# AbrahamSanders/realtime-codec-agent

Measured on NVIDIA B200. Metric: encode audio-sec/sec, higher is better.
Workload: dtype bf16

## Files before the change

### include/magicodec_b200.h

```cpp
#ifndef MAGICODEC_B200_H_
#define MAGICODEC_B200_H_

#include <stdint.h>

#ifdef __cplusplus
extern "C" {
#endif

#define MC_VERSION 100

enum {
  MC_OK = 0,
  MC_ERR_ARG = -1,
  MC_ERR_ARCH = -2,
  MC_ERR_CUDA = -3,
  MC_ERR_STATE = -4,
  MC_ERR_NOMEM = -5
};

typedef struct mc_handle mc_handle;
typedef void* mc_stream_t;

#define MC_MAX_CONVS 8

typedef struct mc_spec {
  int32_t sample_rate;
  int32_t n_convs;
  int32_t conv_channels[MC_MAX_CONVS];
  int32_t conv_strides[MC_MAX_CONVS];
  int32_t d_model, n_heads, ffn_dim;
  int32_t enc_layers, dec_layers;
  int32_t window_left, window_right;
  float norm_eps;
  int32_t codebook_size, codebook_dim;
  int32_t max_positions;
} mc_spec;

int mc_version(void);
const char* mc_last_error(const mc_handle* h);

int mc_create(const mc_spec* spec, int device, mc_handle** out);
int mc_destroy(mc_handle* h);

int mc_set_tensor(mc_handle* h, const char* name, const void* dev_ptr, int64_t numel);
int mc_finalize(mc_handle* h);

int mc_encode(mc_handle* h, const float* wav, int64_t ld, int32_t B, int32_t T, int32_t keep_last_frames,
              int64_t* codes, float* margin, float* z_e, mc_stream_t stream);

int mc_decode(mc_handle* h, const int64_t* codes, int32_t B, int32_t F, int32_t keep_last_samples, float* wav,
              mc_stream_t stream);
int mc_decode_latents(mc_handle* h, const float* z_q, int32_t B, int32_t F, int32_t keep_last_samples,
                      float* wav, mc_stream_t stream);

int mc_vq_search(mc_handle* h, const float* z, int32_t M, int64_t* codes, float* margin, mc_stream_t stream);

int mc_codebook(mc_handle* h, float* out, mc_stream_t stream);

int mc_op_gemm_fused(mc_handle* h, const void* A, const void* W, const float* bias, int32_t M, int32_t N, int32_t K, int32_t act,
                     int32_t out_mode, void* out, const float* row_stats, int32_t row_stats_n, void* xb_out, const float* xb_gamma,
                     float* stat_out, int32_t rope_cols, int32_t rope_period, int32_t block_n, mc_stream_t stream);
int mc_op_rowstats(mc_handle* h, const float* x, const float* gamma, void* xb_out, float* stat_out, int32_t M, int32_t d,
                   mc_stream_t stream);

int64_t mc_debug_trace(mc_handle* h, void* dev_buf, int64_t capacity_records);

enum { MC_PCM_U8 = 0, MC_PCM_S16 = 1, MC_PCM_S24 = 2, MC_PCM_S32 = 3, MC_PCM_F32 = 4, MC_PCM_F64 = 5, MC_PCM_ULAW = 6, MC_PCM_ALAW = 7 };
int mc_op_pcm_to_f32(mc_handle* h, const void* pcm, int32_t format, int32_t big_endian, int32_t channels, int64_t frames,
                     int32_t mix_mono, float* out, int64_t out_ld, mc_stream_t stream);
int mc_op_resample(mc_handle* h, const float* in, int64_t in_ld, int32_t channels, int64_t n_in, int32_t up, int32_t down,
                   const float* taps, int32_t n_taps, int64_t pre_remove, float* out, int64_t out_ld, int64_t n_out,
                   mc_stream_t stream);

int mc_flac_info(const uint8_t* data, int64_t n, int32_t* sample_rate, int32_t* channels, int32_t* bits, int64_t* total_samples);
int mc_flac_decode(const uint8_t* data, int64_t n, void* out, int64_t capacity_frames, int64_t* decoded);

typedef struct mc_stream mc_stream;
int mc_stream_create(mc_handle* h, int32_t channels, int32_t context_samples, int32_t max_chunk_samples, mc_stream** out);
int mc_stream_destroy(mc_stream* s);
int mc_stream_reset(mc_stream* s);
int mc_stream_reset_part(mc_stream* s, int32_t audio, int32_t codes);
int mc_stream_load_audio(mc_stream* s, const float* audio, int32_t n);
int mc_stream_load_codes(mc_stream* s, const int64_t* codes, int32_t n);
int mc_stream_push_audio(mc_stream* s, const float* chunk, int32_t n, int32_t keep_frames, int64_t* codes_out,
                         int32_t* frames_out, mc_stream_t stream);
int mc_stream_push_codes(mc_stream* s, const int64_t* codes, int32_t n, int32_t keep_samples, float* wav_out,
                         int32_t* samples_out, mc_stream_t stream);
int mc_stream_set_graphs(mc_stream* s, int32_t enabled);

typedef struct mc_pool mc_pool;
int mc_pool_create(mc_handle* h, int32_t channels, int32_t context_samples, int32_t max_chunk_samples, int32_t max_sessions,
                   mc_pool** out);
int mc_pool_destroy(mc_pool* p);
int mc_pool_reset(mc_pool* p, int32_t slot, int32_t audio, int32_t codes);
int mc_pool_context_len(mc_pool* p, int32_t slot, int32_t* audio_len, int32_t* code_len);
int mc_pool_set_graphs(mc_pool* p, int32_t enabled);
int mc_pool_push_audio(mc_pool* p, const int32_t* slots, int32_t n, const float* chunks, int32_t len, int32_t keep_frames,
                       int64_t* codes_out, int32_t* frames_out, mc_stream_t stream);
int mc_pool_push_codes(mc_pool* p, const int32_t* slots, int32_t n, const int64_t* codes, int32_t len, int32_t keep_samples,
                       float* wav_out, int32_t* samples_out, mc_stream_t stream);

int mc_stream_set_emit(mc_stream* s, int32_t chunk_samples, int32_t fade_samples, float target_rms,
                       float silence_rms_threshold, const float* fade_in);
int mc_stream_push_codes_emit(mc_stream* s, const int64_t* codes, int32_t n, float* out, int32_t* had_prev,
                              mc_stream_t stream);
int mc_pool_set_emit(mc_pool* p, int32_t chunk_samples, int32_t fade_samples, float target_rms, float silence_rms_threshold,
                     const float* fade_in);
int mc_pool_push_codes_emit(mc_pool* p, const int32_t* slots, int32_t n, const int64_t* codes, int32_t len, float* out,
                            int32_t* had_prev, mc_stream_t stream);

int mc_pool_push_audio_ragged(mc_pool* p, const int32_t* slots, int32_t n, const float* chunks, int32_t len, int32_t keep_frames,
                              int64_t* codes_out, mc_stream_t stream);
int mc_pool_push_codes_ragged(mc_pool* p, const int32_t* slots, int32_t n, const int64_t* codes, int32_t len, int32_t keep_samples,
                              float* wav_out, int32_t* samples_out, mc_stream_t stream);
int mc_pool_push_codes_emit_ragged(mc_pool* p, const int32_t* slots, int32_t n, const int64_t* codes, int32_t len, float* out,
                                   int32_t* had_prev, mc_stream_t stream);
int mc_pool_graph_count(mc_pool* p, int32_t* keys, int32_t* captured);

int mc_embed_distance(mc_handle* h, const int64_t* ids, int32_t rows, int32_t n, int64_t vocab_start, const float* ref,
                      float* dist_out, float* mean_out, mc_stream_t stream);

int64_t mc_launch_count(const mc_handle* h);
int mc_profile_begin(mc_handle* h);
int mc_profile_end(mc_handle* h, double* ms, double* flops, double* bytes, int64_t* launches, int32_t n_classes);
int mc_set_option(mc_handle* h, const char* key, int32_t value);
int mc_set_debug_impl(mc_handle* h, int32_t attention_impl, int32_t vq_impl);


int mc_op_gemm(mc_handle* h, const void* A, int64_t a_rows, int32_t a_k_wrap, const void* W, const float* bias,
               int32_t M, int32_t N, int32_t K, int32_t act, int32_t out_mode, void* out, int64_t ldo,
               int32_t grp_in, int32_t grp_valid, int64_t grp_stride, int64_t grp_off, int32_t rope_cols,
               int32_t rope_period, int32_t block_n, mc_stream_t stream);
int mc_op_rmsnorm(mc_handle* h, const float* x, const float* gamma, void* out_bf16, int32_t M, int32_t d,
                  mc_stream_t stream);
int mc_op_attention(mc_handle* h, const void* qkv, void* out, int32_t B, int32_t F, int32_t out_rows, int32_t phase,
                    int32_t impl, mc_stream_t stream);

int mc_op_emit_chunk(mc_handle* h, const float* wav, int32_t n_have, int32_t chunk, int32_t fade, int32_t has_prev,
                     float target_rms, float silence_rms_threshold, const float* fade_in, float* prev_tail, float* out,
                     mc_stream_t stream);
int mc_op_embed_distance(mc_handle* h, const float* table, int32_t K, const int64_t* ids, int32_t rows, int32_t n,
                         int64_t vocab_start, const float* ref, float* dist_out, float* mean_out, mc_stream_t stream);

int mc_render_chunks(mc_handle* h, const float* windows, int64_t ld, int32_t n_chunks, int32_t chunk, int32_t fade,
                     int32_t last_len, float target_rms, float silence_rms_threshold, const float* fade_in, float* out,
                     mc_stream_t stream);
int mc_op_f32_to_pcm(mc_handle* h, const float* in, int64_t in_ld, int32_t channels, int64_t frames, int32_t format, void* out,
                     mc_stream_t stream);

#ifdef __cplusplus
}
#endif
#endif
```

### realtime-codec-agent_b200/_native.py

```python
from __future__ import annotations

import ctypes as C
import os
from typing import Optional

import torch

from .build import LIB_PATH

MC_MAX_CONVS = 8


class McSpec(C.Structure):
    _fields_ = [
        ("sample_rate", C.c_int32),
        ("n_convs", C.c_int32),
        ("conv_channels", C.c_int32 * MC_MAX_CONVS),
        ("conv_strides", C.c_int32 * MC_MAX_CONVS),
        ("d_model", C.c_int32), ("n_heads", C.c_int32), ("ffn_dim", C.c_int32),
        ("enc_layers", C.c_int32), ("dec_layers", C.c_int32),
        ("window_left", C.c_int32), ("window_right", C.c_int32),
        ("norm_eps", C.c_float),
        ("codebook_size", C.c_int32), ("codebook_dim", C.c_int32),
        ("max_positions", C.c_int32),
    ]


_P, _I32, _I64 = C.c_void_p, C.c_int32, C.c_int64
SYMBOLS = {
    "mc_version": (C.c_int, []),
    "mc_last_error": (C.c_char_p, [_P]),
    "mc_create": (C.c_int, [C.POINTER(McSpec), C.c_int, C.POINTER(_P)]),
    "mc_destroy": (C.c_int, [_P]),
    "mc_set_tensor": (C.c_int, [_P, C.c_char_p, _P, _I64]),
    "mc_finalize": (C.c_int, [_P]),
    "mc_encode": (C.c_int, [_P, _P, _I64, _I32, _I32, _I32, _P, _P, _P, _P]),
    "mc_decode": (C.c_int, [_P, _P, _I32, _I32, _I32, _P, _P]),
    "mc_decode_latents": (C.c_int, [_P, _P, _I32, _I32, _I32, _P, _P]),
    "mc_vq_search": (C.c_int, [_P, _P, _I32, _P, _P, _P]),
    "mc_codebook": (C.c_int, [_P, _P, _P]),
    "mc_launch_count": (_I64, [_P]),
    "mc_debug_trace": (_I64, [_P, _P, _I64]),
    "mc_set_debug_impl": (C.c_int, [_P, _I32, _I32]),
    "mc_set_option": (C.c_int, [_P, C.c_char_p, _I32]),
    "mc_profile_begin": (C.c_int, [_P]),
    "mc_profile_end": (C.c_int, [_P, _P, _P, _P, _P, _I32]),
    "mc_stream_create": (C.c_int, [_P, _I32, _I32, _I32, C.POINTER(_P)]),
    "mc_stream_destroy": (C.c_int, [_P]),
    "mc_stream_reset": (C.c_int, [_P]),
    "mc_stream_reset_part": (C.c_int, [_P, _I32, _I32]),
    "mc_stream_load_audio": (C.c_int, [_P, _P, _I32]),
    "mc_stream_load_codes": (C.c_int, [_P, _P, _I32]),
    "mc_stream_push_audio": (C.c_int, [_P, _P, _I32, _I32, _P, C.POINTER(_I32), _P]),
    "mc_stream_push_codes": (C.c_int, [_P, _P, _I32, _I32, _P, C.POINTER(_I32), _P]),
    "mc_stream_set_graphs": (C.c_int, [_P, _I32]),
    "mc_stream_set_emit": (C.c_int, [_P, _I32, _I32, C.c_float, C.c_float, _P]),
    "mc_stream_push_codes_emit": (C.c_int, [_P, _P, _I32, _P, C.POINTER(_I32), _P]),
    "mc_pool_create": (C.c_int, [_P, _I32, _I32, _I32, _I32, C.POINTER(_P)]),
    "mc_pool_destroy": (C.c_int, [_P]),
    "mc_pool_reset": (C.c_int, [_P, _I32, _I32, _I32]),
    "mc_pool_context_len": (C.c_int, [_P, _I32, C.POINTER(_I32), C.POINTER(_I32)]),
    "mc_pool_set_graphs": (C.c_int, [_P, _I32]),
    "mc_pool_push_audio": (C.c_int, [_P, _P, _I32, _P, _I32, _I32, _P, C.POINTER(_I32), _P]),
    "mc_pool_push_codes": (C.c_int, [_P, _P, _I32, _P, _I32, _I32, _P, C.POINTER(_I32), _P]),
    "mc_pool_set_emit": (C.c_int, [_P, _I32, _I32, C.c_float, C.c_float, _P]),
    "mc_pool_push_codes_emit": (C.c_int, [_P, _P, _I32, _P, _I32, _P, C.POINTER(_I32), _P]),
    "mc_pool_push_audio_ragged": (C.c_int, [_P, _P, _I32, _P, _I32, _I32, _P, _P]),
    "mc_pool_push_codes_ragged": (C.c_int, [_P, _P, _I32, _P, _I32, _I32, _P, _P, _P]),
    "mc_pool_push_codes_emit_ragged": (C.c_int, [_P, _P, _I32, _P, _I32, _P, _P, _P]),
    "mc_pool_graph_count": (C.c_int, [_P, C.POINTER(_I32), C.POINTER(_I32)]),
    "mc_embed_distance": (C.c_int, [_P, _P, _I32, _I32, _I64, _P, _P, _P, _P]),
    "mc_op_gemm": (C.c_int, [_P, _P, _I64, _I32, _P, _P, _I32, _I32, _I32, _I32, _I32, _P, _I64,
                             _I32, _I32, _I64, _I64, _I32, _I32, _I32, _P]),
    "mc_op_emit_chunk": (C.c_int, [_P, _P, _I32, _I32, _I32, _I32, C.c_float, C.c_float, _P, _P, _P, _P]),
    "mc_op_embed_distance": (C.c_int, [_P, _P, _I32, _P, _I32, _I32, _I64, _P, _P, _P, _P]),
    "mc_op_pcm_to_f32": (C.c_int, [_P, _P, _I32, _I32, _I32, _I64, _I32, _P, _I64, _P]),
    "mc_op_resample": (C.c_int, [_P, _P, _I64, _I32, _I64, _I32, _I32, _P, _I32, _I64, _P, _I64, _I64, _P]),
    "mc_render_chunks": (C.c_int, [_P, _P, _I64, _I32, _I32, _I32, _I32, C.c_float, C.c_float, _P, _P, _P]),
    "mc_op_f32_to_pcm": (C.c_int, [_P, _P, _I64, _I32, _I64, _I32, _P, _P]),
    "mc_flac_info": (C.c_int, [_P, _I64, C.POINTER(_I32), C.POINTER(_I32), C.POINTER(_I32), C.POINTER(_I64)]),
    "mc_flac_decode": (C.c_int, [_P, _I64, _P, _I64, C.POINTER(_I64)]),
    "mc_op_gemm_fused": (C.c_int, [_P, _P, _P, _P, _I32, _I32, _I32, _I32, _I32, _P, _P, _I32, _P, _P, _P, _I32, _I32, _I32, _P]),
    "mc_op_rowstats": (C.c_int, [_P, _P, _P, _P, _P, _I32, _I32, _P]),
    "mc_op_rmsnorm": (C.c_int, [_P, _P, _P, _P, _I32, _I32, _P]),
    "mc_op_attention": (C.c_int, [_P, _P, _P, _I32, _I32, _I32, _I32, _I32, _P]),
}

_lib: Optional[C.CDLL] = None


def load_library(path: Optional[str] = None) -> C.CDLL:
    global _lib
    if _lib is not None and path is None:
        return _lib
    path = path or os.environ.get("MAGICODEC_B200_LIB") or LIB_PATH
    if not os.path.isfile(path):
        raise RuntimeError(
            f"{path} is not built. Run `python -c 'import __graft_entry__ as g; g.build()'` "
            "(needs nvcc); the B200 engine has no CPU or PyTorch fallback.")
    lib = C.CDLL(path)
    for name, (res, args) in SYMBOLS.items():
        fn = getattr(lib, name)
        fn.restype, fn.argtypes = res, args
    if lib.mc_version() != 100:
        raise RuntimeError(f"libmagicodec_b200.so version {lib.mc_version()} != header version 100")
    _lib = lib
    return lib


class McError(RuntimeError):
    pass


def check(lib: C.CDLL, handle, rc: int, what: str) -> None:
    if rc != 0:
        msg = lib.mc_last_error(handle)
        raise McError(f"{what} failed (code {rc}): {msg.decode() if msg else '?'}")


def ptr(t: Optional[torch.Tensor]) -> Optional[int]:
    return None if t is None else t.data_ptr()


def current_stream_ptr(device: torch.device) -> int:
    return torch.cuda.current_stream(device).cuda_stream
```

### realtime-codec-agent_b200/build.py

```python
from __future__ import annotations

import hashlib
import os
import shutil
import subprocess
import sys

PKG_DIR = os.path.dirname(os.path.abspath(__file__))
CSRC = os.path.join(PKG_DIR, "csrc")
LIB_NAME = "libmagicodec_b200.so"
LIB_PATH = os.path.join(PKG_DIR, LIB_NAME)
_STAMP = os.path.join(PKG_DIR, ".build_stamp")


def _sources_digest() -> str:
    hsh = hashlib.sha256()
    roots = [CSRC, os.path.join(os.path.dirname(PKG_DIR), "include")]
    for root in roots:
        for name in sorted(os.listdir(root)):
            if name.endswith((".cu", ".cuh", ".h", ".cpp")):
                with open(os.path.join(root, name), "rb") as f:
                    hsh.update(name.encode())
                    hsh.update(f.read())
    return hsh.hexdigest()


def nvcc_path() -> str:
    for cand in (os.environ.get("NVCC"), shutil.which("nvcc"), "/usr/local/cuda/bin/nvcc"):
        if cand and os.path.isfile(cand):
            return cand
    raise RuntimeError("nvcc not found; the B200 engine cannot be built")


def build(force: bool = False, verbose: bool = False, trace: bool = False) -> str:
    digest = _sources_digest() + ("+trace" if trace else "")
    lib_path = LIB_PATH.replace(".so", "_trace.so") if trace else LIB_PATH
    stamp = _STAMP + ("_trace" if trace else "")
    if not force and os.path.isfile(lib_path) and os.path.isfile(stamp):
        with open(stamp) as f:
            if f.read().strip() == digest:
                return lib_path
    cmd = [
        nvcc_path(), "-std=c++17", "-O3", "-lineinfo",
        "-gencode", "arch=compute_100a,code=sm_100a",
        "-Xcompiler", "-fPIC,-O2,-Wall", "-shared", *(["-DMC_TRACE"] if trace else []),
        "-Xptxas", "-v" if verbose else "-O3",
        "-o", lib_path, os.path.join(CSRC, "engine.cu"), os.path.join(CSRC, "audio_decode.cpp"),
        "-lcudart",
    ]
    proc = subprocess.run(cmd, capture_output=True, text=True)
    if verbose or proc.returncode != 0:
        sys.stderr.write(proc.stdout + proc.stderr)
    if proc.returncode != 0:
        raise RuntimeError("nvcc failed building libmagicodec_b200.so:\n" + proc.stderr[-4000:])
    with open(stamp, "w") as f:
        f.write(digest)
    return lib_path


def main(argv=None) -> None:
    argv = sys.argv[1:] if argv is None else argv
    print(build(force="--force" in argv, verbose="-v" in argv, trace="--trace" in argv))


if __name__ == "__main__":
    main()
```

### realtime-codec-agent_b200/csrc/engine.cu

```cuda
#include "engine_common.cuh"

#include "attn_sm100.cuh"
#include "attn_vq_simt.cuh"
#include "elementwise.cuh"
#include "gemm_sm100.cuh"
#include "gemm_splitk_sm100.cuh"
#include "ingest.cuh"
#include "post_sm100.cuh"
#include "vq_sm100.cuh"

using namespace mc;
using namespace mc_internal;

namespace {

struct GemmCall {
  const bf16* A; int64_t a_rows; int a_k_wrap;
  const bf16* W; const float* bias;
  int M, N, K, act, out_mode;
  void* out; int64_t ldo;
  int grp_in = INT_MAX, grp_valid = INT_MAX; int64_t grp_stride = 0, grp_off = 0;
  int rope_cols = 0, rope_period = 0, rope_offset = 0;
  int block_n = 0;
  const void* prefetch_ptr = nullptr;
  long long prefetch_bytes = 0;
  const float* row_stats = nullptr; int row_stats_n = 0;
  bf16* xb_out = nullptr; const float* xb_gamma = nullptr; float* stat_out = nullptr;
};

void fill_norm_fields(const mc_handle* h, const GemmCall& c, GemmParams& p) {
  p.row_stats = c.row_stats; p.row_stats_n = c.row_stats_n;
  p.norm_eps = h->spec.norm_eps; p.inv_norm_dim = c.K > 0 ? 1.0f / (float)c.K : 0.f;
  p.xb_out = c.xb_out; p.xb_gamma = c.xb_gamma; p.stat_out = c.stat_out;
}

template <int BN, int BM = GEMM_BM, int KPS = 1>
int launch_gemm_bn(mc_handle* h, const GemmCall& c, cudaStream_t stream) {
  const CUtensorMap *ma, *mb;
  MC_TRY(get_map_2d_bf16(h, c.A, (uint64_t)c.a_k_wrap, (uint64_t)c.a_rows, GEMM_BK, BM, &ma));
  MC_TRY(get_map_2d_bf16(h, c.W, (uint64_t)c.K, (uint64_t)c.N, GEMM_BK, BN, &mb));
  const bool tma_out = (c.grp_in == INT_MAX) && BM == GEMM_BM && c.xb_out == nullptr;
  const CUtensorMap* mo = ma;
  if (tma_out) {
    const int esize = c.out_mode == OUT_BF16 ? 2 : 4;
    MC_TRY(get_map_2d(h, c.out, esize, (uint64_t)c.N, (uint64_t)c.M, (uint64_t)c.ldo * esize, esize == 2 ? 64 : 32, 32, &mo));
  }
  GemmParams p;
  p.tma_store = tma_out ? 1 : 0;
  p.M = c.M; p.N = c.N; p.K = c.K; p.a_k_wrap = c.a_k_wrap;
  p.bias = c.bias; p.act = c.act; p.out_mode = c.out_mode; p.out = c.out; p.ldo = c.ldo;
  p.grp_in = c.grp_in; p.grp_valid = c.grp_valid; p.grp_stride = c.grp_stride; p.grp_off = c.grp_off;
  p.rope_cols = c.rope_cols; p.rope_period = c.rope_period; p.rope_offset = c.rope_offset;
  p.rope_ld = h->spec.max_positions;
  p.rope_cos = c.rope_period > 0 ? h->ptr<float>("rope.cos") : nullptr;
  p.rope_sin = c.rope_period > 0 ? h->ptr<float>("rope.sin") : nullptr;
  fill_norm_fields(h, c, p);
  MC_TRY(mc_allow_smem(h, (gemm_bf16_sm100_kernel<BN, BM, KPS>), GemmCfg<BN>::kSmemBytes));
  const int m_tiles = (c.M + BM - 1) / BM, n_tiles = (c.N + BN - 1) / BN;
  const int grid = std::min(m_tiles * n_tiles, h->num_sms);
  const double valid_rows = c.grp_in == INT_MAX ? (double)c.M : (double)c.M / c.grp_in * c.grp_valid;
  const double out_bytes = valid_rows * c.N * (c.out_mode == OUT_BF16 ? 2.0 : (c.out_mode == OUT_F32 ? 4.0 : 8.0));
  McProfScope prof(h, 0, 2.0 * valid_rows * c.N * c.K, valid_rows * c.a_k_wrap * 2.0 + (double)c.N * c.K * 2.0 + out_bytes, stream);
  mc_launch(h, gemm_bf16_sm100_kernel<BN, BM, KPS>, dim3(grid), dim3(GEMM_THREADS), GemmCfg<BN>::kSmemBytes, stream, *ma, *mb, *mo, p);
  MC_LAUNCH_CHECK(h, "gemm_bf16_sm100_kernel");
  return MC_OK;
}

template <int EPI>
int launch_gemm_pair_epi(mc_handle* h, const GemmParams& p, const CUtensorMap* ma, const CUtensorMap* mb,
                         const CUtensorMap* mo, const CUtensorMap* mo2, int pairs, cudaStream_t stream) {
  constexpr int BN = 256;
  MC_TRY(mc_allow_smem(h, gemm2_bf16_sm100_kernel<BN, EPI>, Gemm2Cfg<BN, EPI>::kSmemBytes));
  mc_launch(h, gemm2_bf16_sm100_kernel<BN, EPI>, dim3(2 * pairs), dim3(GEMM_THREADS), Gemm2Cfg<BN, EPI>::kSmemBytes, stream, *ma, *mb,
            *mo, *mo2, p);
  MC_LAUNCH_CHECK(h, "gemm2_bf16_sm100_kernel");
  return MC_OK;
}

int launch_gemm_pair(mc_handle* h, const GemmCall& c, cudaStream_t stream) {
  constexpr int BN = 256;
  const CUtensorMap *ma, *mb;
  MC_TRY(get_map_2d_bf16(h, c.A, (uint64_t)c.a_k_wrap, (uint64_t)c.a_rows, GEMM_BK, GEMM_BM, &ma));
  MC_TRY(get_map_2d_bf16(h, c.W, (uint64_t)c.K, (uint64_t)c.N, GEMM_BK, BN / 2, &mb));
  const bool norm_fast = c.xb_out != nullptr && h->fast_epilogue && c.grp_in == INT_MAX && c.bias != nullptr && c.N % BN == 0 &&
                         c.out_mode == OUT_F32_RESIDUAL && c.act == ACT_NONE && c.rope_period == 0 && c.ldo == c.N;
  const bool tma_out = (c.grp_in == INT_MAX) && (c.xb_out == nullptr || norm_fast);
  const CUtensorMap* mo = ma;
  const CUtensorMap* mo2 = ma;
  if (tma_out) {
    const int esize = c.out_mode == OUT_BF16 ? 2 : 4;
    MC_TRY(get_map_2d(h, c.out, esize, (uint64_t)c.N, (uint64_t)c.M, (uint64_t)c.ldo * esize, esize == 2 ? 64 : 32, 32, &mo));
  }
  if (norm_fast) MC_TRY(get_map_2d(h, c.xb_out, 2, (uint64_t)c.N, (uint64_t)c.M, (uint64_t)c.N * 2, 64, 32, &mo2));
  GemmParams p;
  p.tma_store = tma_out ? 1 : 0;
  p.M = c.M; p.N = c.N; p.K = c.K; p.a_k_wrap = c.a_k_wrap;
  p.bias = c.bias; p.act = c.act; p.out_mode = c.out_mode; p.out = c.out; p.ldo = c.ldo;
  p.grp_in = c.grp_in; p.grp_valid = c.grp_valid; p.grp_stride = c.grp_stride; p.grp_off = c.grp_off;
  p.rope_cols = c.rope_cols; p.rope_period = c.rope_period; p.rope_offset = c.rope_offset;
  p.rope_ld = h->spec.max_positions;
  p.rope_cos = c.rope_period > 0 ? h->ptr<float>("rope.cos") : nullptr;
  p.rope_sin = c.rope_period > 0 ? h->ptr<float>("rope.sin") : nullptr;
  fill_norm_fields(h, c, p);
  const int m_tiles = (c.M + 2 * GEMM_BM - 1) / (2 * GEMM_BM), n_tiles = (c.N + BN - 1) / BN;
  const int pairs = std::min(m_tiles * n_tiles, h->num_sms / 2);
  const double valid_rows = c.grp_in == INT_MAX ? (double)c.M : (double)c.M / c.grp_in * c.grp_valid;
  const double out_bytes = valid_rows * c.N * (c.out_mode == OUT_BF16 ? 2.0 : (c.out_mode == OUT_F32 ? 4.0 : 8.0));
  McProfScope prof(h, 0, 2.0 * valid_rows * c.N * c.K, valid_rows * c.a_k_wrap * 2.0 + (double)c.N * c.K * 2.0 + out_bytes, stream);
  const bool fast_ok = h->fast_epilogue && tma_out && c.bias != nullptr && c.N % BN == 0;
  if (norm_fast) return launch_gemm_pair_epi<EPI_RESID_NORM>(h, p, ma, mb, mo, mo2, pairs, stream);
  if (fast_ok && c.out_mode == OUT_BF16 && c.act == ACT_NONE && c.rope_period > 0 && c.rope_cols % 64 == 0)
    return launch_gemm_pair_epi<EPI_ROPE_BF16>(h, p, ma, mb, mo, mo2, pairs, stream);
  if (fast_ok && c.out_mode == OUT_BF16 && c.act == ACT_GELU_TANH && c.rope_period == 0)
    return launch_gemm_pair_epi<EPI_GELU_BF16>(h, p, ma, mb, mo, mo2, pairs, stream);
  if (fast_ok && c.out_mode == OUT_F32_RESIDUAL && c.act == ACT_NONE && c.rope_period == 0 && c.xb_out == nullptr)
    return launch_gemm_pair_epi<EPI_RESID_F32>(h, p, ma, mb, mo, mo2, pairs, stream);
  return launch_gemm_pair_epi<EPI_GENERIC>(h, p, ma, mb, mo, mo2, pairs, stream);
}

template <int S>
int launch_gemm_splitk_s(mc_handle* h, const GemmCall& c, cudaStream_t stream) {
  constexpr int BN = 64;
  const CUtensorMap *ma, *mb;
  MC_TRY(get_map_2d_bf16(h, c.A, (uint64_t)c.a_k_wrap, (uint64_t)c.a_rows, GEMM_BK, GEMM_BM, &ma));
  MC_TRY(get_map_2d_bf16(h, c.W, (uint64_t)c.K, (uint64_t)c.N, GEMM_BK, BN, &mb));
  GemmParams p;
  p.tma_store = 0;
  p.M = c.M; p.N = c.N; p.K = c.K; p.a_k_wrap = c.a_k_wrap;
  p.bias = c.bias; p.act = c.act; p.out_mode = c.out_mode; p.out = c.out; p.ldo = c.ldo;
  p.grp_in = c.grp_in; p.grp_valid = c.grp_valid; p.grp_stride = c.grp_stride; p.grp_off = c.grp_off;
  p.rope_cols = c.rope_cols; p.rope_period = c.rope_period; p.rope_offset = c.rope_offset;
  p.rope_ld = h->spec.max_positions;
  p.rope_cos = c.rope_period > 0 ? h->ptr<float>("rope.cos") : nullptr;
  p.rope_sin = c.rope_period > 0 ? h->ptr<float>("rope.sin") : nullptr;
  if (h->l2_prefetch) { p.prefetch_ptr = c.prefetch_ptr; p.prefetch_bytes = c.prefetch_bytes; }
  fill_norm_fields(h, c, p);
  auto kernel = gemm_splitk_sm100_kernel<BN, S>;
  MC_TRY(mc_allow_smem(h, kernel, GemmSkCfg<BN>::kSmemBytes));
  const int m_tiles = (c.M + GEMM_BM - 1) / GEMM_BM, n_tiles = (c.N + BN - 1) / BN;
  const double valid_rows = c.grp_in == INT_MAX ? (double)c.M : (double)c.M / c.grp_in * c.grp_valid;
  const double out_bytes = valid_rows * c.N * (c.out_mode == OUT_BF16 ? 2.0 : (c.out_mode == OUT_F32 ? 4.0 : 8.0));
  McProfScope prof(h, 0, 2.0 * valid_rows * c.N * c.K, valid_rows * c.a_k_wrap * 2.0 + (double)c.N * c.K * 2.0 + out_bytes, stream);
  cudaLaunchConfig_t cfg = {};
  cfg.gridDim = dim3(m_tiles * n_tiles * S); cfg.blockDim = dim3(GEMM_THREADS);
  cfg.dynamicSmemBytes = GemmSkCfg<BN>::kSmemBytes; cfg.stream = stream;
  cudaLaunchAttribute at[2];
  at[0].id = cudaLaunchAttributeClusterDimension;
  at[0].val.clusterDim.x = S; at[0].val.clusterDim.y = 1; at[0].val.clusterDim.z = 1;
  at[1].id = cudaLaunchAttributeProgrammaticStreamSerialization;
  at[1].val.programmaticStreamSerializationAllowed = 1;
  cfg.attrs = at;
  cfg.numAttrs = h->pdl ? 2 : 1;
  const int nkb = (c.K / GEMM_BK) / S;
  const int kps = 1;
  (void)nkb;
  (void)cudaLaunchKernelEx(&cfg, kernel, *ma, *mb, p, kps);
  MC_LAUNCH_CHECK(h, "gemm_splitk_sm100_kernel");
  return MC_OK;
}

int pick_split_k(const mc_handle* h, const GemmCall& c) {
  if (c.M > 2 * GEMM_BM) return 0;
  const int base = ((c.M + GEMM_BM - 1) / GEMM_BM) * ((c.N + 63) / 64);
  const int num_kb = c.K / GEMM_BK;
  if (base > 32) {
    if (base <= 48 && num_kb >= 32 && num_kb % 4 == 0) return 4;
    return 0;
  }
  for (int s = 8; s >= 2; s >>= 1)
    if (num_kb % s == 0 && num_kb / s >= 2 && base * s <= h->num_sms) return s;
  return 0;
}

int launch_gemm_splitk(mc_handle* h, const GemmCall& c, int S, cudaStream_t stream) {
  if (c.rope_period > 0 && c.rope_cols % 64 != 0) return h->fail(MC_ERR_ARG, "split-K gemm: rope needs 64-wide heads");
  if ((c.K / GEMM_BK) % S != 0) return h->fail(MC_ERR_ARG, "split-K gemm: %d k-blocks do not split %d ways", c.K / GEMM_BK, S);
  switch (S) {
    case 2: return launch_gemm_splitk_s<2>(h, c, stream);
    case 4: return launch_gemm_splitk_s<4>(h, c, stream);
    case 8: return launch_gemm_splitk_s<8>(h, c, stream);
    default: return h->fail(MC_ERR_ARG, "split-K gemm: unsupported split %d", S);
  }
}

int launch_gemm(mc_handle* h, const GemmCall& c, cudaStream_t stream) {
  if (c.K % GEMM_BK != 0 || c.K % c.a_k_wrap != 0 || c.a_k_wrap % GEMM_BK != 0)
    return h->fail(MC_ERR_ARG, "gemm: K=%d a_k_wrap=%d must be multiples of %d", c.K, c.a_k_wrap, GEMM_BK);
  if (c.N % 8 != 0) return h->fail(MC_ERR_ARG, "gemm: N=%d must be a multiple of 8", c.N);
  if (c.rope_period > 0 && c.rope_period + c.rope_offset > h->spec.max_positions)
    return h->fail(MC_ERR_ARG, "gemm: rope period %d exceeds table rows %d", c.rope_period, h->spec.max_positions);
  int bn = c.block_n;
  if (c.xb_out && (c.out_mode == OUT_BF16 || c.N % 64 != 0 || !c.xb_gamma || !c.stat_out))
    return h->fail(MC_ERR_ARG, "gemm: fused RMSNorm producer needs an fp32 output, N %% 64 == 0, gamma and a stats buffer");
  if (bn >= 1002 && bn <= 1008) return launch_gemm_splitk(h, c, bn - 1000, stream);
  if (bn == 4064 && (c.K / GEMM_BK) % 4 == 0) return launch_gemm_bn<64, GEMM_BM, 4>(h, c, stream);
  if (bn == 0 && (h->split_k == 2 || (h->split_k == 1 && h->in_session))) {
    const int S = pick_split_k(h, c);
    if (S >= 2) return launch_gemm_splitk(h, c, S, stream);
  }
  {
    const int m2 = (c.M + 255) / 256, n2 = (c.N + 255) / 256;
    if ((bn == 0 && h->gemm_pair && c.N >= 256 && m2 * n2 >= h->num_sms / 2) || bn == 512) return launch_gemm_pair(h, c, stream);
  }
  if (bn == 0) {
    const int m_tiles = (c.M + GEMM_BM - 1) / GEMM_BM;
    if (c.N >= 256 && m_tiles * ((c.N + 255) / 256) >= 2 * h->num_sms) bn = 256;
    else if (c.N >= 128 && m_tiles * ((c.N + 127) / 128) >= h->num_sms) bn = 128;
    else if (c.N >= 256 && m_tiles * ((c.N + 255) / 256) >= h->num_sms) bn = 256;
    else bn = 64;
  }
  if (bn == 64 && c.block_n == 0 && (c.K / GEMM_BK) % 4 == 0 &&
      ((c.M + GEMM_BM - 1) / GEMM_BM) * ((c.N + 63) / 64) <= h->num_sms)
    return launch_gemm_bn<64, GEMM_BM, 4>(h, c, stream);
  switch (bn) {
    case 256: return launch_gemm_bn<256>(h, c, stream);
    case 128: return launch_gemm_bn<128>(h, c, stream);
    case 64: return launch_gemm_bn<64>(h, c, stream);
    default: return h->fail(MC_ERR_ARG, "gemm: unsupported block_n %d", bn);
  }
}

int ew_grid(mc_handle* h, long long work_items, int threads) {
  long long blocks = (work_items + threads - 1) / threads;
  const long long cap = (long long)h->num_sms * 16;
  if (blocks > cap) blocks = cap;
  if (blocks < 1) blocks = 1;
  return (int)blocks;
}

int launch_rmsnorm(mc_handle* h, const float* x, const float* gamma, bf16* out, int M, int d, int grp_in,
                   int64_t grp_stride, int64_t grp_off, cudaStream_t stream) {
  if (d % 4 != 0) return h->fail(MC_ERR_ARG, "rmsnorm: d=%d must be a multiple of 4", d);
  const int warps = 8;
  const int grid = ew_grid(h, M, warps);
  McProfScope prof(h, 3, 0.0, (double)M * d * 6.0, stream);
  const float eps = h->spec.norm_eps;
  switch (d % 128 == 0 ? d / 128 : 0) {
    case 1: mc_launch(h, rmsnorm_rows_kernel<1>, dim3(grid), dim3(warps * 32), 0, stream, x, gamma, out, M, eps, grp_in, (long long)grp_stride, (long long)grp_off); break;
    case 2: mc_launch(h, rmsnorm_rows_kernel<2>, dim3(grid), dim3(warps * 32), 0, stream, x, gamma, out, M, eps, grp_in, (long long)grp_stride, (long long)grp_off); break;
    case 4: mc_launch(h, rmsnorm_rows_kernel<4>, dim3(grid), dim3(warps * 32), 0, stream, x, gamma, out, M, eps, grp_in, (long long)grp_stride, (long long)grp_off); break;
    case 8: mc_launch(h, rmsnorm_rows_kernel<8>, dim3(grid), dim3(warps * 32), 0, stream, x, gamma, out, M, eps, grp_in, (long long)grp_stride, (long long)grp_off); break;
    default: mc_launch(h, rmsnorm_kernel, dim3(grid), dim3(warps * 32), 0, stream, x, gamma, out, M, d, eps, grp_in, (long long)grp_stride, (long long)grp_off);
  }
  MC_LAUNCH_CHECK(h, "rmsnorm_kernel");
  return MC_OK;
}

int launch_attention(mc_handle* h, const bf16* qkv, bf16* out, int B, int F, int out_rows, int phase, int impl, cudaStream_t stream) {
  if (out_rows < 1 || out_rows > F) return h->fail(MC_ERR_ARG, "attention: out_rows %d not in 1 .. %d", out_rows, F);
  const mc_spec& s = h->spec;
  const double span = std::min(F, s.window_left + s.window_right + 1);
  McProfScope prof(h, 1, 4.0 * B * out_rows * span * s.d_model,
                   (double)B * (F * 2.0 + out_rows * 2.0) * s.d_model * 2.0, stream);
  if (impl == 0 && attn_sm100_supported(s.window_left, s.window_right)) {
    MC_TRY(launch_attention_sm100_v3(h, qkv, out, B, F, out_rows, phase, stream));
    return MC_OK;
  }
  if (impl != 0 && impl != 1) return h->fail(MC_ERR_ARG, "attention: unknown implementation %d (0 = tcgen05, 1 = SIMT cross-check)", impl);
  if (s.window_left + s.window_right + 1 > 160) return h->fail(MC_ERR_ARG, "attention window too wide");
  const long long warps = (long long)B * F * s.n_heads;
  const int threads = 256;
  const long long blocks = (warps * 32 + threads - 1) / threads;
  attention_window_simt_kernel<<<(unsigned)blocks, threads, 0, stream>>>(qkv, out, B, F, s.n_heads, s.window_left,
                                                                         s.window_right, out_rows, 0.125f);
  MC_LAUNCH_CHECK(h, "attention_window_simt_kernel");
  return MC_OK;
}

struct StackBufs {
  float* x;
  float* x2;
  bf16* hbuf;
  bf16* qkv;
  bf16* att;
  bf16* ffn;
  float* stats;
};

bool few_rows_regime(const mc_handle* h, long long M) {
  return (h->split_k == 2 || (h->split_k == 1 && h->in_session)) && M <= 2 * GEMM_BM;
}
bool fuse_norm_ok(const mc_handle* h, long long M) {
  if (h->spec.d_model % 64 != 0 || h->fuse_norm == 0) return false;
  return h->fuse_norm >= 2 || few_rows_regime(h, M);
}

int launch_rowstats(mc_handle* h, const float* x, const float* gamma, bf16* xb, float* stats, long long M, int d, cudaStream_t stream) {
  McProfScope prof(h, 3, 0.0, (double)M * d * 6.0, stream);
  mc_launch(h, rowstats_cast_kernel, dim3(ew_grid(h, M * (d / 64), 256)), dim3(256), 0, stream, x, gamma, xb, stats, M, d);
  MC_LAUNCH_CHECK(h, "rowstats_cast_kernel");
  return MC_OK;
}

int run_layers(mc_handle* h, const char* prefix, int n_layers, const StackBufs& b, int B, int F, int keep_rows,
               float** x_out, cudaStream_t stream, int fuse_mode = 0 ,
               const float* final_gamma = nullptr, bf16** xb_out = nullptr, float** stats_out = nullptr) {
  const mc_spec& s = h->spec;
  const int d = s.d_model, f = s.ffn_dim;
  const int nst = d / 64;
  const bool fused = fuse_mode == 1;
  const bool fused2 = fuse_mode != 0;
  std::vector<int> r_in(n_layers), r_out(n_layers);
  {
    int need = std::max(1, std::min(keep_rows, F));
    if (B == 1 && F <= GEMM_BM) need = F;
    for (int l = n_layers - 1; l >= 0; --l) {
      r_out[l] = need;
      need = (need >= F) ? F : std::min(F, need + s.window_left);
      if (!h->exact_cut && need < F) need = F - ((F - need) / 16) * 16;
      r_in[l] = need;
    }
  }
  float* x = b.x;
  float* xalt = b.x2;
  int rows = F;
  char name[128];
  for (int l = 0; l < n_layers; ++l) {
    auto T = [&](const char* leaf) {
      snprintf(name, sizeof(name), "%s.layers.%d.%s", prefix, l, leaf);
      return std::string(name);
    };
    const int Ri = rows, Ro = std::min(r_out[l], rows);
    const int Mi = B * Ri, Mo = B * Ro;
    if (!fused) MC_TRY(launch_rmsnorm(h, x, h->ptr<float>(T("norm1")), b.hbuf, Mi, d, INT_MAX, 0, 0, stream));
    GemmCall g{};
    if (fused) { g.row_stats = b.stats; g.row_stats_n = nst; }
    g.A = b.hbuf; g.a_rows = Mi; g.a_k_wrap = d; g.W = h->ptr<bf16>(T("wqkv")); g.bias = h->ptr<float>(T("bqkv"));
    g.M = Mi; g.N = 3 * d; g.K = d; g.act = ACT_NONE; g.out_mode = OUT_BF16; g.out = b.qkv; g.ldo = 3 * d;
    g.rope_cols = 2 * d; g.rope_period = Ri; g.rope_offset = F - Ri;
    g.prefetch_ptr = h->ptr<bf16>(T("wo")); g.prefetch_bytes = (long long)d * d * 2;
    MC_TRY(launch_gemm(h, g, stream));
    MC_TRY(launch_attention(h, b.qkv, b.att, B, Ri, Ro, (F - Ri) % 16, h->attn_impl, stream));
    if (Ro < Ri) {
      const long long items = (long long)Mo * (d / 4);
      McProfScope prof(h, 3, 0.0, (double)Mo * d * 8.0, stream);
      mc_launch(h, compact_rows_kernel, dim3(ew_grid(h, items, 256)), dim3(256), 0, stream, reinterpret_cast<const float4*>(x),
                reinterpret_cast<float4*>(xalt), B, Ri, Ro, d / 4);
      MC_LAUNCH_CHECK(h, "compact_rows_kernel");
      std::swap(x, xalt);
      rows = Ro;
    }
    GemmCall o{};
    o.A = b.att; o.a_rows = Mo; o.a_k_wrap = d; o.W = h->ptr<bf16>(T("wo")); o.bias = h->ptr<float>(T("bo"));
    o.M = Mo; o.N = d; o.K = d; o.act = ACT_NONE; o.out_mode = OUT_F32_RESIDUAL; o.out = x; o.ldo = d;
    o.prefetch_ptr = h->ptr<bf16>(T("w1")); o.prefetch_bytes = (long long)f * d * 2;
    if (fused2) { o.xb_out = b.hbuf; o.xb_gamma = h->ptr<float>(T("norm2")); o.stat_out = b.stats; }
    MC_TRY(launch_gemm(h, o, stream));
    if (!fused2) MC_TRY(launch_rmsnorm(h, x, h->ptr<float>(T("norm2")), b.hbuf, Mo, d, INT_MAX, 0, 0, stream));
    GemmCall u{};
    if (fused2) { u.row_stats = b.stats; u.row_stats_n = nst; }
    u.A = b.hbuf; u.a_rows = Mo; u.a_k_wrap = d; u.W = h->ptr<bf16>(T("w1")); u.bias = h->ptr<float>(T("b1"));
    u.M = Mo; u.N = f; u.K = d; u.act = ACT_GELU_TANH; u.out_mode = OUT_BF16; u.out = b.ffn; u.ldo = f;
    u.prefetch_ptr = h->ptr<bf16>(T("w2")); u.prefetch_bytes = (long long)d * f * 2;
    MC_TRY(launch_gemm(h, u, stream));
    GemmCall w{};
    w.A = b.ffn; w.a_rows = Mo; w.a_k_wrap = f; w.W = h->ptr<bf16>(T("w2")); w.bias = h->ptr<float>(T("b2"));
    w.M = Mo; w.N = d; w.K = f; w.act = ACT_NONE; w.out_mode = OUT_F32_RESIDUAL; w.out = x; w.ldo = d;
    if (l + 1 < n_layers) {
      snprintf(name, sizeof(name), "%s.layers.%d.wqkv", prefix, l + 1);
      w.prefetch_ptr = h->ptr<bf16>(name); w.prefetch_bytes = (long long)3 * d * d * 2;
    }
    if (fused) {
      const float* next_gamma = final_gamma;
      if (l + 1 < n_layers) {
        snprintf(name, sizeof(name), "%s.layers.%d.norm1", prefix, l + 1);
        next_gamma = h->ptr<float>(name);
      }
      if (next_gamma) { w.xb_out = b.hbuf; w.xb_gamma = next_gamma; w.stat_out = b.stats; }
    }
    MC_TRY(launch_gemm(h, w, stream));
  }
  bf16* xb = b.hbuf;
  float* st = b.stats;
  if (rows > keep_rows && B == 1) {
    x += (size_t)(rows - keep_rows) * d;
    xb += (size_t)(rows - keep_rows) * d;
    st += (size_t)(rows - keep_rows) * nst;
  } else if (rows > keep_rows) {
    const int Ro = keep_rows;
    const long long items = (long long)B * Ro * (d / 4);
    mc_launch(h, compact_rows_kernel, dim3(ew_grid(h, items, 256)), dim3(256), 0, stream, reinterpret_cast<const float4*>(x),
              reinterpret_cast<float4*>(xalt), B, rows, Ro, d / 4);
    MC_LAUNCH_CHECK(h, "compact_rows_kernel");
    std::swap(x, xalt);
  }
  if (fused && final_gamma && rows > keep_rows && B != 1) return h->fail(MC_ERR_STATE, "run_layers: fused norms with a trailing compaction");
  *x_out = x;
  if (xb_out) *xb_out = xb;
  if (stats_out) *stats_out = st;
  return MC_OK;
}

StackBufs carve_stack(Carver& cv, uint8_t* base, int M, int d, int f, bool dry) {
  StackBufs b{};
  size_t ox = cv.take((size_t)M * d * 4), ox2 = cv.take((size_t)M * d * 4), oh = cv.take((size_t)M * d * 2),
         oq = cv.take((size_t)M * 3 * d * 2), oa = cv.take((size_t)M * d * 2), of = cv.take((size_t)M * f * 2),
         os = cv.take((size_t)M * (d / 64 + 1) * 4);
  if (!dry) {
    b.stats = reinterpret_cast<float*>(base + os);
    b.x = reinterpret_cast<float*>(base + ox);
    b.x2 = reinterpret_cast<float*>(base + ox2);
    b.hbuf = reinterpret_cast<bf16*>(base + oh);
    b.qkv = reinterpret_cast<bf16*>(base + oq);
    b.att = reinterpret_cast<bf16*>(base + oa);
    b.ffn = reinterpret_cast<bf16*>(base + of);
  }
  return b;
}

int launch_vq(mc_handle* h, const float* z, int n_items, int F, int keep, int64_t* codes, float* margin,
              void* scratch, cudaStream_t stream);
size_t vq_scratch_bytes(mc_handle* h, int Mq);

struct ConvPlan {
  int B = 0, T = 0;
  std::vector<int> Tl;
  std::vector<size_t> off;
};

// ... 231 lines not shown
  MC_TRY(launch_gemm(h, ip, stream));
  if (fused && !proj_producer) MC_TRY(launch_rowstats(h, sb.x, h->ptr<float>("dec.layers.0.norm1"), sb.hbuf, sb.stats, M, d, stream));
  float* xk = nullptr;
  MC_TRY(run_layers(h, "dec", s.dec_layers, sb, B, F, Rk, &xk, stream, fuse_mode));

  {
    PadList pl;
    long long work = 0;
    for (int i = 0; i < n; ++i) {
      pl.base[pl.n] = base + tb_off[i];
      pl.pitch[pl.n] = (long long)(1 + Tin[i]) * dch[i] * 2;
      pl.width[pl.n] = dch[i] * 2;
      if (pl.width[pl.n] % 16 != 0) return h->fail(MC_ERR_ARG, "tconv %d: %d channels are not 16-byte granular", i, dch[i]);
      work = std::max(work, (long long)B * (pl.width[pl.n] >> 4));
      ++pl.n;
    }
    mc_launch(h, zero_pads_kernel, dim3(ew_grid(h, work, 256)), dim3(256), 0, stream, pl, B);
    MC_LAUNCH_CHECK(h, "zero_pads_kernel");
  }
  MC_TRY(launch_rmsnorm(h, xk, h->ptr<float>("dec.norm_f"), reinterpret_cast<bf16*>(base + tb_off[0]), B * Rk, d, Rk,
                        (int64_t)(1 + Rk) * d, d, stream));
  for (int i = 0; i + 1 < n; ++i) {
    GemmCall g{};
    g.A = reinterpret_cast<const bf16*>(base + tb_off[i]);
    g.a_k_wrap = dch[i]; g.a_rows = (int64_t)B * (1 + Tin[i]);
    g.W = h->ptr<bf16>("dec.up" + std::to_string(i) + ".w");
    g.bias = h->ptr<float>("dec.up" + std::to_string(i) + ".b");
    g.M = B * (1 + Tin[i]); g.N = ds[i] * dch[i + 1]; g.K = 2 * dch[i];
    g.grp_in = 1 + Tin[i]; g.grp_valid = Tin[i];
    g.act = ACT_GELU_TANH; g.out_mode = OUT_BF16; g.out = base + tb_off[i + 1]; g.ldo = g.N;
    g.grp_stride = (int64_t)(1 + Tin[i + 1]) * dch[i + 1]; g.grp_off = dch[i + 1];
    MC_TRY(launch_gemm(h, g, stream));
  }
  {
    const int i = n - 1;
    if (ds[i] > 8 || dch[i] % 8 != 0) return h->fail(MC_ERR_ARG, "last tconv: stride %d / channels %d unsupported", ds[i], dch[i]);
    const long long items = (long long)B * Tin[i];
    const size_t smem = (size_t)dch[i] * 2 * ds[i] * 4;
    McProfScope prof(h, 3, 4.0 * B * Tin[i] * dch[i] * ds[i], (double)B * Tin[i] * dch[i] * 2.0 + (double)B * keep * 4.0, stream);
    mc_launch(h, tconv_last_kernel<8>, dim3(ew_grid(h, items, threads)), dim3(threads), smem, stream,
              reinterpret_cast<const bf16*>(base + tb_off[i]), B, Tin[i], dch[i], ds[i],
              h->ptr<float>("dec.up" + std::to_string(i) + ".w"), h->ptr<float>("dec.up" + std::to_string(i) + ".b"), wav, keep);
    MC_LAUNCH_CHECK(h, "tconv_last_kernel");
  }
  return MC_OK;
}

size_t vq_scratch_bytes(mc_handle* h, int Mq) {
  return std::max(vq_sm100_scratch_bytes(h->num_sms, Mq), (size_t)64 * Mq * sizeof(VqPartial)) + 1024;
}

int launch_vq(mc_handle* h, const float* z, int n_items, int F, int keep, int64_t* codes, float* margin,
              void* scratch, cudaStream_t stream) {
  const mc_spec& s = h->spec;
  const int Mq = n_items * keep;
  McProfScope prof(h, 2, 2.0 * Mq * (double)s.codebook_size * s.codebook_dim, (double)s.codebook_size * 128.0, stream);
  if (h->vq_impl == 0) {
    return launch_vq_sm100(h, z, n_items, F, keep, codes, margin, scratch, stream);
  }
  const int row_tiles = (Mq + 127) / 128;
  int splits = (2 * h->num_sms + row_tiles - 1) / row_tiles;
  splits = std::max(1, std::min(64, splits));
  vq_simt_kernel<<<dim3(row_tiles, splits), 128, 0, stream>>>(z, Mq, F, keep, h->ptr<float>("vq.codebook"),
                                                              h->ptr<float>("vq.c2"), s.codebook_size, splits,
                                                              reinterpret_cast<VqPartial*>(scratch));
  MC_LAUNCH_CHECK(h, "vq_simt_kernel");
  vq_merge_kernel<<<(Mq + 255) / 256, 256, 0, stream>>>(reinterpret_cast<const VqPartial*>(scratch), Mq, splits,
                                                        reinterpret_cast<long long*>(codes), margin);
  MC_LAUNCH_CHECK(h, "vq_merge_kernel");
  return MC_OK;
}

std::vector<std::string> required_tensors(const mc_spec& s) {
  std::vector<std::string> v;
  const int n = s.n_convs;
  for (int i = 0; i < n; ++i) {
    v.push_back("enc.conv" + std::to_string(i) + ".w");
    v.push_back("enc.conv" + std::to_string(i) + ".b");
    v.push_back("dec.up" + std::to_string(i) + ".w");
    v.push_back("dec.up" + std::to_string(i) + ".b");
  }
  const char* leaves[] = {"norm1", "wqkv", "bqkv", "wo", "bo", "norm2", "w1", "b1", "w2", "b2"};
  for (int st = 0; st < 2; ++st)
    for (int l = 0; l < (st == 0 ? s.enc_layers : s.dec_layers); ++l)
      for (const char* leaf : leaves)
        v.push_back(std::string(st == 0 ? "enc" : "dec") + ".layers." + std::to_string(l) + "." + leaf);
  for (const char* nm : {"enc.norm_f", "enc.proj.w", "enc.proj.b", "vq.codebook", "vq.c2", "vq.packed", "dec.in_proj.w",
                         "dec.in_proj.b", "dec.norm_f", "rope.cos", "rope.sin"})
    v.push_back(nm);
  return v;
}

}

extern "C" {

int mc_version(void) { return MC_VERSION; }

const char* mc_last_error(const mc_handle* h) { return h ? h->err.c_str() : g_create_error.c_str(); }

int mc_create(const mc_spec* spec, int device, mc_handle** out) {
  if (!spec || !out) { g_create_error = "mc_create: null argument"; return MC_ERR_ARG; }
  *out = nullptr;
  cudaDeviceProp prop;
  cudaError_t e = cudaGetDeviceProperties(&prop, device);
  if (e != cudaSuccess) { g_create_error = std::string("mc_create: ") + cudaGetErrorString(e); return MC_ERR_CUDA; }
  if (prop.major != 10) {
    g_create_error = "mc_create: device is sm_" + std::to_string(prop.major * 10 + prop.minor) +
                     "; this library contains sm_100a code only (no fallback)";
    return MC_ERR_ARCH;
  }
  if (spec->n_convs < 2 || spec->n_convs > MC_MAX_CONVS || spec->d_model % 64 != 0 || spec->d_model / spec->n_heads != 64 ||
      spec->ffn_dim % 64 != 0 || spec->codebook_dim != 16 || spec->codebook_size % 256 != 0 ||
      spec->conv_channels[spec->n_convs - 1] != spec->d_model) {
    g_create_error = "mc_create: unsupported spec (need head_dim 64, d/ffn multiples of 64, codebook_dim 16)";
    return MC_ERR_ARG;
  }
  e = cudaSetDevice(device);
  if (e != cudaSuccess) { g_create_error = std::string("mc_create: ") + cudaGetErrorString(e); return MC_ERR_CUDA; }
  mc_handle* h = new mc_handle();
  h->spec = *spec;
  h->device = device;
  h->num_sms = prop.multiProcessorCount;
  *out = h;
  return MC_OK;
}

int mc_destroy(mc_handle* h) {
  if (!h) return MC_OK;
  if (h->arena) cudaFree(h->arena);
  delete h;
  return MC_OK;
}

int mc_set_tensor(mc_handle* h, const char* name, const void* dev_ptr, int64_t numel) {
  if (!h || !name || !dev_ptr) return MC_ERR_ARG;
  Tensor t; t.p = dev_ptr; t.numel = numel;
  h->tensors[name] = t;
  h->tensor_gen++;
  h->finalized = false;
  return MC_OK;
}

int mc_finalize(mc_handle* h) {
  if (!h) return MC_ERR_ARG;
  for (const std::string& nm : required_tensors(h->spec))
    if (!h->find(nm)) return h->fail(MC_ERR_ARG, "mc_finalize: tensor '%s' was not registered", nm.c_str());
  h->finalized = true;
  return MC_OK;
}

#define MC_ENTER(h)                                                        \
  if (!(h)) return MC_ERR_ARG;                                             \
  if (!(h)->finalized) return (h)->fail(MC_ERR_STATE, "handle not finalized"); \
  { cudaError_t e__ = cudaSetDevice((h)->device); if (e__ != cudaSuccess) return (h)->fail(MC_ERR_CUDA, "cudaSetDevice failed"); }

int mc_encode(mc_handle* h, const float* wav, int64_t ld, int32_t B, int32_t T, int32_t keep_last_frames,
              int64_t* codes, float* margin, float* z_e, mc_stream_t stream) {
  MC_ENTER(h);
  if (!wav || !codes || B < 1 || T < 1) return h->fail(MC_ERR_ARG, "mc_encode: bad arguments (B=%d T=%d)", B, T);
  return encode_impl(h, wav, ld, B, T, keep_last_frames, codes, margin, z_e, (cudaStream_t)stream);
}

int mc_decode(mc_handle* h, const int64_t* codes, int32_t B, int32_t F, int32_t keep_last_samples, float* wav,
              mc_stream_t stream) {
  MC_ENTER(h);
  if (!codes || !wav) return h->fail(MC_ERR_ARG, "mc_decode: null pointer");
  return decode_impl(h, codes, nullptr, B, F, keep_last_samples, wav, (cudaStream_t)stream);
}

int mc_decode_latents(mc_handle* h, const float* z_q, int32_t B, int32_t F, int32_t keep_last_samples, float* wav,
                      mc_stream_t stream) {
  MC_ENTER(h);
  if (!z_q || !wav) return h->fail(MC_ERR_ARG, "mc_decode_latents: null pointer");
  return decode_impl(h, nullptr, z_q, B, F, keep_last_samples, wav, (cudaStream_t)stream);
}

int mc_vq_search(mc_handle* h, const float* z, int32_t M, int64_t* codes, float* margin, mc_stream_t stream) {
  MC_ENTER(h);
  if (!z || !codes || M < 1) return h->fail(MC_ERR_ARG, "mc_vq_search: bad arguments");
  Carver cv;
  cv.take(vq_scratch_bytes(h, M));
  MC_TRY(arena_reserve(h, cv.off, (cudaStream_t)stream));
  return launch_vq(h, z, M, 1, 1, codes, margin, h->arena, (cudaStream_t)stream);
}

int mc_codebook(mc_handle* h, float* out, mc_stream_t stream) {
  MC_ENTER(h);
  const Tensor* t = h->find("vq.codebook");
  MC_CUDA(h, cudaMemcpyAsync(out, t->p, (size_t)t->numel * 4, cudaMemcpyDeviceToDevice, (cudaStream_t)stream));
  return MC_OK;
}

int mc_embed_distance(mc_handle* h, const int64_t* ids, int32_t rows, int32_t n, int64_t vocab_start, const float* ref,
                      float* dist_out, float* mean_out, mc_stream_t stream) {
  MC_ENTER(h);
  if (!ids || rows < 1 || n < 1 || (!dist_out && !mean_out)) return h->fail(MC_ERR_ARG, "mc_embed_distance: bad arguments");
  embed_distance_kernel<<<rows, POST_THREADS, 0, (cudaStream_t)stream>>>(
      reinterpret_cast<const long long*>(ids), n, (long long)vocab_start, h->ptr<float>("vq.codebook"), h->spec.codebook_size,
      ref, dist_out, mean_out);
  MC_LAUNCH_CHECK(h, "embed_distance_kernel");
  return MC_OK;
}

int mc_op_embed_distance(mc_handle* h, const float* table, int32_t K, const int64_t* ids, int32_t rows, int32_t n,
                         int64_t vocab_start, const float* ref, float* dist_out, float* mean_out, mc_stream_t stream) {
  MC_ENTER(h);
  if (!table || K < 1 || !ids || rows < 1 || n < 1 || (!dist_out && !mean_out))
    return h->fail(MC_ERR_ARG, "mc_op_embed_distance: bad arguments");
  embed_distance_kernel<<<rows, POST_THREADS, 0, (cudaStream_t)stream>>>(reinterpret_cast<const long long*>(ids), n,
                                                                         (long long)vocab_start, table, K, ref, dist_out, mean_out);
  MC_LAUNCH_CHECK(h, "embed_distance_kernel");
  return MC_OK;
}

int mc_op_emit_chunk(mc_handle* h, const float* wav, int32_t n_have, int32_t chunk, int32_t fade, int32_t has_prev,
                     float target_rms, float silence_rms_threshold, const float* fade_in, float* prev_tail, float* out,
                     mc_stream_t stream) {
  MC_ENTER(h);
  if (!wav || !fade_in || !prev_tail || !out || chunk < 1 || fade < 1 || fade > chunk || n_have < 1)
    return h->fail(MC_ERR_ARG, "mc_op_emit_chunk: bad arguments");
  emit_chunk_kernel<<<1, POST_THREADS, 0, (cudaStream_t)stream>>>(wav, n_have, chunk, fade, has_prev, target_rms,
                                                                  silence_rms_threshold, fade_in, prev_tail, out);
  MC_LAUNCH_CHECK(h, "emit_chunk_kernel");
  return MC_OK;
}

int mc_render_chunks(mc_handle* h, const float* windows, int64_t ld, int32_t n_chunks, int32_t chunk, int32_t fade,
                     int32_t last_len, float target_rms, float silence_rms_threshold, const float* fade_in, float* out,
                     mc_stream_t stream) {
  MC_ENTER(h);
  if (!windows || !fade_in || !out || n_chunks < 1 || chunk < 1 || fade < 1 || fade > chunk || last_len < 1 || last_len > chunk ||
      ld < (int64_t)chunk + fade)
    return h->fail(MC_ERR_ARG, "mc_render_chunks: need 0 < fade (%d) <= chunk (%d), 0 < last_len (%d) <= chunk, ld (%lld) >= chunk + fade",
                   fade, chunk, last_len, (long long)ld);
  const double out_n = (double)(n_chunks - 1) * chunk + last_len;
  McProfScope prof(h, 3, 0.0, out_n * 4.0 * 2.0 + (double)n_chunks * fade * 4.0, (cudaStream_t)stream);
  mc_launch(h, emit_chunks_kernel, dim3(n_chunks), dim3(POST_THREADS), 0, (cudaStream_t)stream, windows, (long long)ld, (int)n_chunks,
            (int)chunk, (int)fade, (int)last_len, target_rms, silence_rms_threshold, fade_in, out);
  MC_LAUNCH_CHECK(h, "emit_chunks_kernel");
  return MC_OK;
}

int mc_op_f32_to_pcm(mc_handle* h, const float* in, int64_t in_ld, int32_t channels, int64_t frames, int32_t format, void* out,
                     mc_stream_t stream) {
  MC_ENTER(h);
  if (!in || !out || channels < 1 || frames < 1 || in_ld < frames || (format != PCM_S16 && format != PCM_F32))
    return h->fail(MC_ERR_ARG, "mc_op_f32_to_pcm: bad arguments (format %d, channels %d, frames %lld)", format, channels, (long long)frames);
  if (reinterpret_cast<uintptr_t>(out) & (format == PCM_S16 ? 1 : 3))
    return h->fail(MC_ERR_ARG, "mc_op_f32_to_pcm: output is not naturally aligned");
  McProfScope prof(h, 3, 0.0, (double)frames * channels * (4.0 + (format == PCM_S16 ? 2.0 : 4.0)), (cudaStream_t)stream);
  f32_to_pcm_kernel<<<ew_grid(h, frames * channels, 256), 256, 0, (cudaStream_t)stream>>>(in, (long long)in_ld, channels,
                                                                                          (long long)frames, format, out);
  MC_LAUNCH_CHECK(h, "f32_to_pcm_kernel");
  return MC_OK;
}

int mc_op_pcm_to_f32(mc_handle* h, const void* pcm, int32_t format, int32_t big_endian, int32_t channels, int64_t frames,
                     int32_t mix_mono, float* out, int64_t out_ld, mc_stream_t stream) {
  MC_ENTER(h);
  if (!pcm || !out || channels < 1 || frames < 1 || format < PCM_U8 || format > PCM_ALAW || (!mix_mono && out_ld < frames))
    return h->fail(MC_ERR_ARG, "mc_op_pcm_to_f32: bad arguments (format %d, channels %d, frames %lld)", format, channels, (long long)frames);
  if ((format == PCM_F32 && (reinterpret_cast<uintptr_t>(pcm) & 3)) || (format == PCM_F64 && (reinterpret_cast<uintptr_t>(pcm) & 7)))
    return h->fail(MC_ERR_ARG, "mc_op_pcm_to_f32: float payload is not naturally aligned");
  McProfScope prof(h, 3, 0.0, (double)frames * channels * 2.0 + (double)frames * (mix_mono ? 1 : channels) * 4.0, (cudaStream_t)stream);
  pcm_to_f32_kernel<<<ew_grid(h, frames, 256), 256, 0, (cudaStream_t)stream>>>(
      reinterpret_cast<const unsigned char*>(pcm), format, big_endian, channels, (long long)frames, mix_mono, out, (long long)out_ld);
  MC_LAUNCH_CHECK(h, "pcm_to_f32_kernel");
  return MC_OK;
}

int mc_op_resample(mc_handle* h, const float* in, int64_t in_ld, int32_t channels, int64_t n_in, int32_t up, int32_t down,
                   const float* taps, int32_t n_taps, int64_t pre_remove, float* out, int64_t out_ld, int64_t n_out,
                   mc_stream_t stream) {
  MC_ENTER(h);
  if (!in || !taps || !out || channels < 1 || n_in < 1 || n_out < 1 || up < 1 || down < 1 || n_taps < 1 || pre_remove < 0 ||
      in_ld < n_in || out_ld < n_out)
    return h->fail(MC_ERR_ARG, "mc_op_resample: bad arguments (up %d, down %d, taps %d)", up, down, n_taps);
  McProfScope prof(h, 3, 2.0 * channels * (double)n_out * ((double)n_taps / up), (double)channels * (n_in + n_out) * 4.0, (cudaStream_t)stream);
  resample_poly_kernel<<<ew_grid(h, (long long)channels * n_out, 256), 256, 0, (cudaStream_t)stream>>>(
      in, (long long)in_ld, channels, (long long)n_in, up, down, taps, n_taps, (long long)pre_remove, out, (long long)out_ld,
      (long long)n_out);
  MC_LAUNCH_CHECK(h, "resample_poly_kernel");
  return MC_OK;
}

int64_t mc_debug_trace(mc_handle* h, void* dev_buf, int64_t capacity_records) {
  if (!h) return MC_ERR_ARG;
#ifdef MC_TRACE
  unsigned int n = 0, zero = 0, cap = (unsigned int)capacity_records;
  cudaDeviceSynchronize();
  cudaMemcpyFromSymbol(&n, g_mc_trace_n, sizeof(n));
  unsigned long long* ptr = reinterpret_cast<unsigned long long*>(dev_buf);
  cudaMemcpyToSymbol(g_mc_trace, &ptr, sizeof(ptr));
  cudaMemcpyToSymbol(g_mc_trace_cap, &cap, sizeof(cap));
  cudaMemcpyToSymbol(g_mc_trace_n, &zero, sizeof(zero));
  return (int64_t)n;
#else
  (void)dev_buf; (void)capacity_records;
  return h->fail(MC_ERR_STATE, "mc_debug_trace: the library was built without -DMC_TRACE");
#endif
}

int64_t mc_launch_count(const mc_handle* h) { return h ? h->launches : 0; }

int mc_profile_begin(mc_handle* h) {
  if (!h) return MC_ERR_ARG;
  for (auto& r : h->prof) { h->event_pool.push_back(r.a); h->event_pool.push_back(r.b); }
  h->prof.clear();
  h->profiling = true;
  return MC_OK;
}

int mc_profile_end(mc_handle* h, double* ms, double* flops, double* bytes, int64_t* launches, int32_t n_classes) {
  if (!h || !ms || !flops || !bytes || !launches) return MC_ERR_ARG;
  h->profiling = false;
  for (int c = 0; c < n_classes; ++c) { ms[c] = 0; flops[c] = 0; bytes[c] = 0; launches[c] = 0; }
  for (auto& r : h->prof) {
    cudaError_t e = cudaEventSynchronize(r.b);
    if (e != cudaSuccess) return h->fail(MC_ERR_CUDA, "mc_profile_end: %s", cudaGetErrorString(e));
    float t = 0.f;
    cudaEventElapsedTime(&t, r.a, r.b);
    if (r.cls < n_classes) { ms[r.cls] += t; flops[r.cls] += r.flops; bytes[r.cls] += r.bytes; launches[r.cls]++; }
    h->event_pool.push_back(r.a); h->event_pool.push_back(r.b);
  }
  h->prof.clear();
  return MC_OK;
}

int mc_set_option(mc_handle* h, const char* key, int32_t value) {
  if (!h || !key) return MC_ERR_ARG;
  const std::string k(key);
  if (k == "shared_stem") h->shared_stem = value != 0;
  else if (k == "exact_cut") { h->exact_cut = value != 0; h->tensor_gen++; }
  else if (k == "gemm_pair") h->gemm_pair = value != 0;
  else if (k == "fast_epilogue") h->fast_epilogue = value != 0;
  else if (k == "pdl") h->pdl = value != 0;
  else if (k == "attn_p_tmem") h->attn_p_tmem = value != 0;
  else if (k == "debug_repeat") h->debug_repeat = value;
  else if (k == "l2_prefetch") { h->l2_prefetch = value != 0; h->tensor_gen++; }
  else if (k == "fuse_norm") {
    if (value < 0 || value > 3) return h->fail(MC_ERR_ARG, "mc_set_option: fuse_norm is 0 .. 3");
    h->fuse_norm = value; h->tensor_gen++;
  }
  else if (k == "small_m_split_k") {
    if (value < 0 || value > 2) return h->fail(MC_ERR_ARG, "mc_set_option: small_m_split_k is 0, 1 or 2");
    h->split_k = value;
    h->tensor_gen++;
  }
  else if (k == "max_positions") {
    if (value < 1) return h->fail(MC_ERR_ARG, "mc_set_option: max_positions must be positive");
    h->spec.max_positions = value;
  }
  else return h->fail(MC_ERR_ARG, "mc_set_option: unknown option '%s'", key);
  return MC_OK;
}

int mc_set_debug_impl(mc_handle* h, int32_t attention_impl, int32_t vq_impl) {
  if (!h) return MC_ERR_ARG;
  h->gemm_pair = (attention_impl & 4) ? 0 : 1;
  attention_impl &= 1;
  h->attn_impl = attention_impl;
  h->vq_impl = vq_impl;
  return MC_OK;
}

int mc_op_gemm(mc_handle* h, const void* A, int64_t a_rows, int32_t a_k_wrap, const void* W, const float* bias,
               int32_t M, int32_t N, int32_t K, int32_t act, int32_t out_mode, void* out, int64_t ldo,
               int32_t grp_in, int32_t grp_valid, int64_t grp_stride, int64_t grp_off, int32_t rope_cols,
               int32_t rope_period, int32_t block_n, mc_stream_t stream) {
  MC_ENTER(h);
  GemmCall g{};
  g.A = reinterpret_cast<const bf16*>(A); g.a_rows = a_rows; g.a_k_wrap = a_k_wrap;
  g.W = reinterpret_cast<const bf16*>(W); g.bias = bias; g.M = M; g.N = N; g.K = K; g.act = act; g.out_mode = out_mode;
  g.out = out; g.ldo = ldo;
  g.grp_in = grp_in > 0 ? grp_in : INT_MAX; g.grp_valid = grp_in > 0 ? grp_valid : INT_MAX;
  g.grp_stride = grp_stride; g.grp_off = grp_off;
  g.rope_cols = rope_cols; g.rope_period = rope_period; g.block_n = block_n;
  for (int r = 1; r < h->debug_repeat; ++r) MC_TRY(launch_gemm(h, g, (cudaStream_t)stream));
  return launch_gemm(h, g, (cudaStream_t)stream);
}

int mc_op_gemm_fused(mc_handle* h, const void* A, const void* W, const float* bias, int32_t M, int32_t N, int32_t K, int32_t act,
                     int32_t out_mode, void* out, const float* row_stats, int32_t row_stats_n, void* xb_out, const float* xb_gamma,
                     float* stat_out, int32_t rope_cols, int32_t rope_period, int32_t block_n, mc_stream_t stream) {
  MC_ENTER(h);
  GemmCall g{};
  g.A = reinterpret_cast<const bf16*>(A); g.a_rows = M; g.a_k_wrap = K;
  g.W = reinterpret_cast<const bf16*>(W); g.bias = bias; g.M = M; g.N = N; g.K = K; g.act = act; g.out_mode = out_mode;
  g.out = out; g.ldo = N;
  g.rope_cols = rope_cols; g.rope_period = rope_period; g.block_n = block_n;
  g.row_stats = row_stats; g.row_stats_n = row_stats_n;
  g.xb_out = reinterpret_cast<bf16*>(xb_out); g.xb_gamma = xb_gamma; g.stat_out = stat_out;
  for (int r = 1; r < h->debug_repeat; ++r) MC_TRY(launch_gemm(h, g, (cudaStream_t)stream));
  return launch_gemm(h, g, (cudaStream_t)stream);
}

int mc_op_rowstats(mc_handle* h, const float* x, const float* gamma, void* xb_out, float* stat_out, int32_t M, int32_t d,
                   mc_stream_t stream) {
  MC_ENTER(h);
  if (!x || !gamma || !xb_out || !stat_out || M < 1 || d % 64 != 0) return h->fail(MC_ERR_ARG, "mc_op_rowstats: bad arguments");
  for (int r = 1; r < h->debug_repeat; ++r) MC_TRY(launch_rowstats(h, x, gamma, reinterpret_cast<bf16*>(xb_out), stat_out, M, d, (cudaStream_t)stream));
  return launch_rowstats(h, x, gamma, reinterpret_cast<bf16*>(xb_out), stat_out, M, d, (cudaStream_t)stream);
}

int mc_op_rmsnorm(mc_handle* h, const float* x, const float* gamma, void* out_bf16, int32_t M, int32_t d,
                  mc_stream_t stream) {
  MC_ENTER(h);
  for (int r = 1; r < h->debug_repeat; ++r) MC_TRY(launch_rmsnorm(h, x, gamma, reinterpret_cast<bf16*>(out_bf16), M, d, INT_MAX, 0, 0, (cudaStream_t)stream));
  return launch_rmsnorm(h, x, gamma, reinterpret_cast<bf16*>(out_bf16), M, d, INT_MAX, 0, 0, (cudaStream_t)stream);
}

int mc_op_attention(mc_handle* h, const void* qkv, void* out, int32_t B, int32_t F, int32_t out_rows, int32_t phase,
                    int32_t impl, mc_stream_t stream) {
  MC_ENTER(h);
  for (int r = 1; r < h->debug_repeat; ++r)
    MC_TRY(launch_attention(h, reinterpret_cast<const bf16*>(qkv), reinterpret_cast<bf16*>(out), B, F, out_rows, phase, impl,
                            (cudaStream_t)stream));
  return launch_attention(h, reinterpret_cast<const bf16*>(qkv), reinterpret_cast<bf16*>(out), B, F, out_rows, phase, impl,
                          (cudaStream_t)stream);
}

}

struct mc_stream {
  mc_handle* h = nullptr;
  int C = 1;
  int ctx_samples = 32000, ctx_frames = 100;
  int cap_samples = 0, cap_frames = 0;
  float* audio[2] = {nullptr, nullptr};
  int64_t* codes_ctx[2] = {nullptr, nullptr};
  int audio_len = 0, code_len = 0, acur = 0, ccur = 0;
  int32_t* pin_table = nullptr;
  float* pin_audio = nullptr;
  int64_t* pin_codes = nullptr;
  float* pin_wav = nullptr;
  int64_t* dev_codes_out = nullptr;
  float* dev_wav_out = nullptr;
  struct GraphEntry { cudaGraphExec_t exec = nullptr; int uses = 0; size_t arena_gen = 0; };
  std::map<std::tuple<int, int, int, int, int>, GraphEntry> graphs;
  bool use_graphs = true;
  cudaStream_t own = nullptr;
  cudaEvent_t order_ev = nullptr;
  std::string err;
  int emit_chunk = 0, emit_fade = 0, emit_has_prev = 0;
  float emit_target_rms = 0.f, emit_silence_thr = 0.f;
  float* emit_fade_in = nullptr;
  float* emit_prev_tail = nullptr;
  float* emit_out = nullptr;
  float* pin_emit = nullptr;
};

namespace {

size_t handle_generation(const mc_handle* h) {
  return reinterpret_cast<size_t>(h->arena) ^ h->arena_cap ^ (static_cast<size_t>(h->tensor_gen) << 48);
}

void stream_drop_graphs(mc_stream* s) {
  for (auto& kv : s->graphs)
    if (kv.second.exec) cudaGraphExecDestroy(kv.second.exec);
  s->graphs.clear();
}

template <typename Sess, typename Key, typename Body>
int run_or_replay_impl(Sess* s, Key key, cudaStream_t stream, Body body);

template <typename Sess, typename Key, typename Body>
int run_or_replay(Sess* s, Key key, cudaStream_t stream, Body body) {
  s->h->in_session = true;
  const int rc = run_or_replay_impl(s, key, stream, body);
  s->h->in_session = false;
  return rc;
}

template <typename Sess, typename Key, typename Body>
int run_or_replay_impl(Sess* s, Key key, cudaStream_t stream, Body body) {
  mc_handle* h = s->h;
  if (!s->use_graphs || h->profiling) return body();
  auto& e = s->graphs[key];
  const size_t gen = handle_generation(h);
  if (e.exec && e.arena_gen != gen) {
    cudaGraphExecDestroy(e.exec);
    e.exec = nullptr;
    e.uses = 0;
  }
  if (e.exec) {
    MC_CUDA(h, cudaGraphLaunch(e.exec, stream));
    h->launches += 1;
    return MC_OK;
  }
  if (e.uses++ == 0) return body();
  MC_CUDA(h, cudaStreamBeginCapture(stream, cudaStreamCaptureModeRelaxed));
  const int64_t launches_before = h->launches;
  const int rc = body();
  cudaGraph_t graph = nullptr;
  cudaError_t ce = cudaStreamEndCapture(stream, &graph);
  h->launches = launches_before;
  if (rc != MC_OK || ce != cudaSuccess || graph == nullptr) {
    if (graph) cudaGraphDestroy(graph);
    (void)cudaGetLastError();
    s->use_graphs = false;
    return body();
  }
  ce = cudaGraphInstantiate(&e.exec, graph, 0);
  cudaGraphDestroy(graph);
  if (ce != cudaSuccess) {
    e.exec = nullptr;
    s->use_graphs = false;
    return body();
  }
  e.arena_gen = handle_generation(h);
  MC_CUDA(h, cudaGraphLaunch(e.exec, stream));
  h->launches += 1;
  return MC_OK;
}

}

extern "C" {

int mc_stream_create(mc_handle* h, int32_t channels, int32_t context_samples, int32_t max_chunk_samples, mc_stream** out) {
  MC_ENTER(h);
  if (!out || channels < 1 || context_samples < 1) return h->fail(MC_ERR_ARG, "mc_stream_create: bad arguments");
  int hop = 1;
  for (int i = 0; i < h->spec.n_convs; ++i) hop *= h->spec.conv_strides[i];
  mc_stream* s = new mc_stream();
  s->h = h; s->C = channels;
  s->ctx_samples = context_samples;
  s->ctx_frames = context_samples / hop;
  s->cap_samples = std::max(context_samples, max_chunk_samples);
  s->cap_frames = (s->cap_samples + hop - 1) / hop;
  if (s->cap_frames > h->spec.max_positions) { delete s; return h->fail(MC_ERR_ARG, "mc_stream_create: context exceeds RoPE table"); }
  const size_t ab = (size_t)channels * s->cap_samples * 4, cb = (size_t)channels * s->cap_frames * 8;
  cudaError_t e = cudaSuccess;
  for (int i = 0; i < 2 && e == cudaSuccess; ++i) {
    e = cudaMalloc(&s->audio[i], ab);
    if (e == cudaSuccess) e = cudaMalloc(&s->codes_ctx[i], cb);
  }
  if (e == cudaSuccess) e = cudaMalloc(&s->dev_codes_out, cb);
  if (e == cudaSuccess) e = cudaMalloc(&s->dev_wav_out, ab);
  if (e == cudaSuccess) e = cudaMallocHost(&s->pin_table, 16);
  if (e == cudaSuccess) e = cudaMallocHost(&s->pin_audio, ab);
  if (e == cudaSuccess) e = cudaMallocHost(&s->pin_codes, cb);
  if (e == cudaSuccess) e = cudaMallocHost(&s->pin_wav, ab);
  if (e == cudaSuccess) e = cudaStreamCreateWithFlags(&s->own, cudaStreamNonBlocking);
  if (e == cudaSuccess) e = cudaEventCreateWithFlags(&s->order_ev, cudaEventDisableTiming);
  if (e != cudaSuccess) { mc_stream_destroy(s); return h->fail(MC_ERR_NOMEM, "mc_stream_create: %s", cudaGetErrorString(e)); }
  *out = s;
  return MC_OK;
}

int mc_stream_destroy(mc_stream* s) {
  if (!s) return MC_OK;
  stream_drop_graphs(s);
  for (int i = 0; i < 2; ++i) { if (s->audio[i]) cudaFree(s->audio[i]); if (s->codes_ctx[i]) cudaFree(s->codes_ctx[i]); }
  if (s->dev_codes_out) cudaFree(s->dev_codes_out);
  if (s->dev_wav_out) cudaFree(s->dev_wav_out);
  if (s->pin_table) cudaFreeHost(s->pin_table);
  if (s->pin_audio) cudaFreeHost(s->pin_audio);
  if (s->pin_codes) cudaFreeHost(s->pin_codes);
  if (s->pin_wav) cudaFreeHost(s->pin_wav);
  if (s->emit_fade_in) cudaFree(s->emit_fade_in);
  if (s->emit_prev_tail) cudaFree(s->emit_prev_tail);
  if (s->emit_out) cudaFree(s->emit_out);
  if (s->pin_emit) cudaFreeHost(s->pin_emit);
  if (s->order_ev) cudaEventDestroy(s->order_ev);
  if (s->own) cudaStreamDestroy(s->own);
  delete s;
  return MC_OK;
}

int mc_stream_reset(mc_stream* s) {
  if (!s) return MC_ERR_ARG;
  s->audio_len = 0; s->code_len = 0;
  s->emit_has_prev = 0;
  return MC_OK;
}

int mc_stream_reset_part(mc_stream* s, int32_t audio, int32_t codes) {
  if (!s) return MC_ERR_ARG;
  if (audio) s->audio_len = 0;
  if (codes) s->code_len = 0;
  return MC_OK;
}

int mc_stream_load_audio(mc_stream* s, const float* audio, int32_t n) {
  if (!s) return MC_ERR_ARG;
  mc_handle* h = s->h;
  MC_ENTER(h);
  if (n < 0 || (n > 0 && !audio)) return h->fail(MC_ERR_ARG, "mc_stream_load_audio: bad arguments");
  const int keep = std::min(n, s->ctx_samples);
  MC_CUDA(h, cudaStreamSynchronize(s->own));
  if (keep > 0)
    MC_CUDA(h, cudaMemcpy2D(s->audio[s->acur], (size_t)s->cap_samples * 4, audio + (n - keep), (size_t)n * 4, (size_t)keep * 4,
                            s->C, cudaMemcpyHostToDevice));
  s->audio_len = keep;
  return MC_OK;
}

int mc_stream_load_codes(mc_stream* s, const int64_t* codes, int32_t n) {
  if (!s) return MC_ERR_ARG;
  mc_handle* h = s->h;
  MC_ENTER(h);
  if (n < 0 || (n > 0 && !codes)) return h->fail(MC_ERR_ARG, "mc_stream_load_codes: bad arguments");
  const int keep = std::min(n, s->ctx_frames);
  MC_CUDA(h, cudaStreamSynchronize(s->own));
  if (keep > 0)
    MC_CUDA(h, cudaMemcpy2D(s->codes_ctx[s->ccur], (size_t)s->cap_frames * 8, codes + (n - keep), (size_t)n * 8, (size_t)keep * 8,
                            s->C, cudaMemcpyHostToDevice));
  s->code_len = keep;
  return MC_OK;
}

int mc_stream_push_audio(mc_stream* s, const float* chunk, int32_t n, int32_t keep_frames, int64_t* codes_out,
                         int32_t* frames_out, mc_stream_t stream_) {
  if (!s) return MC_ERR_ARG;
  mc_handle* h = s->h;
  MC_ENTER(h);
  cudaStream_t caller = (cudaStream_t)stream_;
  MC_CUDA(h, cudaEventRecord(s->order_ev, caller));
  MC_CUDA(h, cudaStreamWaitEvent(s->own, s->order_ev, 0));
  cudaStream_t stream = s->own;
  if (!chunk || !codes_out || n < 1) return h->fail(MC_ERR_ARG, "mc_stream_push_audio: bad arguments");
  if (n > s->cap_samples) return h->fail(MC_ERR_ARG, "mc_stream_push_audio: chunk of %d samples exceeds the session capacity %d", n, s->cap_samples);
  int hop = 1;
  for (int i = 0; i < h->spec.n_convs; ++i) hop *= h->spec.conv_strides[i];
  const int C = s->C, cap = s->cap_samples;
  const int new_len = std::min(s->audio_len + n, std::max(n, s->ctx_samples));
  const int keep_old = new_len - n;
  const int F = (new_len + hop - 1) / hop;
  const int keep = (keep_frames <= 0 || keep_frames > F) ? F : keep_frames;
  for (int c = 0; c < C; ++c) memcpy(s->pin_audio + (size_t)c * cap, chunk + (size_t)c * n, (size_t)n * 4);
  const int src = s->acur, dst = s->acur ^ 1;
  const int old_len = s->audio_len;
  s->pin_table[0] = 0; s->pin_table[1] = src;
  auto body = [&]() -> int {
    pool_roll_kernel<float><<<dim3((new_len + 255) / 256, C), 256, 0, stream>>>(s->pin_table, C, cap, old_len, keep_old, n, s->audio[0],
                                                                               s->audio[1], s->pin_audio, nullptr, 0);
// ... 637 lines not shown
```

### realtime-codec-agent_b200/csrc/engine_common.cuh

```cuda
#pragma once
#include <cuda.h>
#include <cuda_runtime.h>
#include <stdarg.h>
#include <stdio.h>
#include <string.h>

#include <algorithm>
#include <climits>
#include <map>
#include <set>
#include <string>
#include <tuple>
#include <unordered_map>
#include <utility>
#include <vector>

#include "../../include/magicodec_b200.h"
#include "ptx_sm100.cuh"

typedef __nv_bfloat16 bf16;

namespace mc_internal {

inline thread_local std::string g_create_error;

typedef CUresult (*EncodeTiledFn)(CUtensorMap*, CUtensorMapDataType, cuuint32_t, void*, const cuuint64_t*,
                                  const cuuint64_t*, const cuuint32_t*, const cuuint32_t*, CUtensorMapInterleave,
                                  CUtensorMapSwizzle, CUtensorMapL2promotion, CUtensorMapFloatOOBfill);

inline EncodeTiledFn get_encode_fn() {
  static EncodeTiledFn fn = nullptr;
  if (fn == nullptr) {
    void* p = nullptr;
    cudaDriverEntryPointQueryResult q;
    if (cudaGetDriverEntryPoint("cuTensorMapEncodeTiled", &p, cudaEnableDefault, &q) == cudaSuccess &&
        q == cudaDriverEntryPointSuccess) {
      fn = reinterpret_cast<EncodeTiledFn>(p);
    }
  }
  return fn;
}

struct Tensor {
  const void* p = nullptr;
  int64_t numel = 0;
};

}
using mc_internal::Tensor;

struct mc_handle {
  mc_spec spec{};
  int device = 0;
  int num_sms = 148;
  bool finalized = false;
  std::unordered_map<std::string, Tensor> tensors;
  std::string err;
  int64_t launches = 0;
  uint32_t tensor_gen = 0;
  int attn_impl = 0, vq_impl = 0;
  int gemm_pair = 1;
  bool fast_epilogue = true;
  bool attn_p_tmem = true;
  int split_k = 1;
  bool in_session = false;
  int debug_repeat = 1;
  int fuse_norm = 1;
  bool l2_prefetch = true;
  bool pdl = true;
  bool shared_stem = true;
  bool exact_cut = true;
  struct ProfRec { cudaEvent_t a, b; int cls; double flops; double bytes; };
  bool profiling = false;
  std::vector<ProfRec> prof;
  std::vector<cudaEvent_t> event_pool;
  std::set<const void*> smem_configured;
  uint8_t* arena = nullptr;
  size_t arena_cap = 0;
  size_t arena_off = 0;
  std::map<std::tuple<const void*, uint64_t, uint64_t, uint64_t, uint32_t, uint32_t>, CUtensorMap> maps;

  int fail(int code, const char* fmt, ...) {
    char buf[1024];
    va_list ap;
    va_start(ap, fmt);
    vsnprintf(buf, sizeof(buf), fmt, ap);
    va_end(ap);
    err = buf;
    return code;
  }
  const Tensor* find(const std::string& name) const {
    auto it = tensors.find(name);
    return it == tensors.end() ? nullptr : &it->second;
  }
  template <typename T>
  const T* ptr(const std::string& name) const {
    return reinterpret_cast<const T*>(tensors.at(name).p);
  }
};

#define MC_CUDA(h, expr)                                                                         \
  do {                                                                                           \
    cudaError_t e__ = (expr);                                                                    \
    if (e__ != cudaSuccess)                                                                      \
      return (h)->fail(MC_ERR_CUDA, "%s failed: %s (%s:%d)", #expr, cudaGetErrorString(e__), __FILE__, __LINE__); \
  } while (0)
#define MC_TRY(expr)          \
  do {                        \
    int rc__ = (expr);        \
    if (rc__ != MC_OK) return rc__; \
  } while (0)
struct McProfScope {
  mc_handle* h; cudaStream_t st; bool on;
  mc_handle::ProfRec rec;
  static cudaEvent_t get_event(mc_handle* h) {
    if (!h->event_pool.empty()) { cudaEvent_t e = h->event_pool.back(); h->event_pool.pop_back(); return e; }
    cudaEvent_t e; cudaEventCreate(&e); return e;
  }
  McProfScope(mc_handle* h_, int cls, double flops, double bytes, cudaStream_t s) : h(h_), st(s), on(h_->profiling) {
    if (!on) return;
    rec.a = get_event(h); rec.b = get_event(h); rec.cls = cls; rec.flops = flops; rec.bytes = bytes;
    cudaEventRecord(rec.a, st);
  }
  ~McProfScope() {
    if (!on) return;
    cudaEventRecord(rec.b, st);
    h->prof.push_back(rec);
  }
};

template <typename K>
inline int mc_allow_smem(mc_handle* h, K kernel, int bytes) {
  const void* key = reinterpret_cast<const void*>(kernel);
  if (h->smem_configured.count(key)) return MC_OK;
  MC_CUDA(h, cudaFuncSetAttribute(kernel, cudaFuncAttributeMaxDynamicSharedMemorySize, bytes));
  h->smem_configured.insert(key);
  return MC_OK;
}

template <typename... P, typename... A>
inline void mc_launch(mc_handle* h, void (*kernel)(P...), dim3 grid, dim3 block, size_t smem, cudaStream_t stream, A&&... args) {
  cudaLaunchConfig_t cfg = {};
  cfg.gridDim = grid; cfg.blockDim = block; cfg.dynamicSmemBytes = smem; cfg.stream = stream;
  cudaLaunchAttribute at[1];
  at[0].id = cudaLaunchAttributeProgrammaticStreamSerialization;
  at[0].val.programmaticStreamSerializationAllowed = 1;
  cfg.attrs = at;
  cfg.numAttrs = h->pdl ? 1 : 0;
  (void)cudaLaunchKernelEx(&cfg, kernel, std::forward<A>(args)...);
}

#define MC_LAUNCH_CHECK(h, what)                                                                  \
  do {                                                                                            \
    cudaError_t e__ = cudaGetLastError();                                                         \
    if (e__ != cudaSuccess) return (h)->fail(MC_ERR_CUDA, "launch of %s failed: %s", what, cudaGetErrorString(e__)); \
    (h)->launches++;                                                                              \
  } while (0)

namespace mc_internal {

inline int arena_reserve(mc_handle* h, size_t bytes, cudaStream_t stream) {
  if (bytes <= h->arena_cap) return MC_OK;
  MC_CUDA(h, cudaStreamSynchronize(stream));
  if (h->arena) MC_CUDA(h, cudaFree(h->arena));
  h->arena = nullptr;
  h->arena_cap = 0;
  h->maps.clear();
  const size_t cap = bytes + bytes / 8 + (1u << 20);
  cudaError_t e = cudaMalloc(&h->arena, cap);
  if (e != cudaSuccess) return h->fail(MC_ERR_NOMEM, "workspace cudaMalloc(%zu) failed: %s", cap, cudaGetErrorString(e));
  h->arena_cap = cap;
  return MC_OK;
}
struct Carver {
  size_t off = 0;
  size_t take(size_t bytes) {
    const size_t at = off;
    off += (bytes + 1023) & ~size_t(1023);
    return at;
  }
};

inline int get_map_2d(mc_handle* h, const void* base, int esize, uint64_t dim0, uint64_t dim1, uint64_t row_stride_bytes,
                      uint32_t box0, uint32_t box1, const CUtensorMap** out, int swizzle_bytes = 128) {
  auto key = std::make_tuple(base, dim0, dim1, row_stride_bytes, (uint32_t)(box0 | (esize << 16) | (swizzle_bytes << 20)), box1);
  auto it = h->maps.find(key);
  if (it != h->maps.end()) {
    *out = &it->second;
    return MC_OK;
  }
  EncodeTiledFn enc = get_encode_fn();
  if (!enc) return h->fail(MC_ERR_CUDA, "cuTensorMapEncodeTiled entry point not available");
  if ((reinterpret_cast<uintptr_t>(base) & 15) != 0 || row_stride_bytes % 16 != 0 || box0 * esize > (uint32_t)swizzle_bytes)
    return h->fail(MC_ERR_ARG, "TMA operand misaligned (base %p, row stride %llu B, box %u x %d B)", base,
                   (unsigned long long)row_stride_bytes, box0, esize);
  CUtensorMap m;
  cuuint64_t gdim[2] = {dim0, dim1};
  cuuint64_t gstride[1] = {row_stride_bytes};
  cuuint32_t box[2] = {box0, box1};
  cuuint32_t estride[2] = {1, 1};
  CUresult r = enc(&m, esize == 2 ? CU_TENSOR_MAP_DATA_TYPE_BFLOAT16 : CU_TENSOR_MAP_DATA_TYPE_FLOAT32, 2,
                   const_cast<void*>(base), gdim, gstride, box, estride, CU_TENSOR_MAP_INTERLEAVE_NONE,
                   swizzle_bytes == 32 ? CU_TENSOR_MAP_SWIZZLE_32B : CU_TENSOR_MAP_SWIZZLE_128B, CU_TENSOR_MAP_L2_PROMOTION_L2_256B,
                   CU_TENSOR_MAP_FLOAT_OOB_FILL_NONE);
  if (r != CUDA_SUCCESS)
    return h->fail(MC_ERR_CUDA, "cuTensorMapEncodeTiled failed (%d) dims %llu x %llu box %u x %u esize %d", (int)r,
                   (unsigned long long)dim0, (unsigned long long)dim1, box0, box1, esize);
  auto ins = h->maps.emplace(key, m);
  *out = &ins.first->second;
  return MC_OK;
}
inline int get_map_2d_bf16(mc_handle* h, const void* base, uint64_t dim0, uint64_t dim1, uint32_t box0, uint32_t box1,
                           const CUtensorMap** out, int swizzle_bytes = 128) {
  return get_map_2d(h, base, 2, dim0, dim1, dim0 * 2, box0, box1, out, swizzle_bytes);
}
}
```

### realtime-codec-agent_b200/csrc/gemm_sm100.cuh

```cuda
#pragma once
#include <type_traits>

#include "ptx_sm100.cuh"

namespace mc {

enum : int { ACT_NONE = 0, ACT_GELU_TANH = 1 };
enum : int { OUT_BF16 = 0, OUT_F32 = 1, OUT_F32_RESIDUAL = 2 };

struct GemmParams {
  int M, N, K;
  int a_k_wrap;
  const float* bias;
  int act;
  int out_mode;
  void* out;
  long long ldo;
  int grp_in, grp_valid;
  long long grp_stride, grp_off;
  int tma_store;
  const float* rope_cos;
  int rope_ld;
  const float* rope_sin;
  int rope_cols;
  int rope_period;
  int rope_offset;
  int one = 1;
  const void* prefetch_ptr = nullptr;
  long long prefetch_bytes = 0;
  const float* row_stats = nullptr;
  int row_stats_n = 0;
  float norm_eps = 0.f, inv_norm_dim = 0.f;
  __nv_bfloat16* xb_out = nullptr;
  const float* xb_gamma = nullptr;
  float* stat_out = nullptr;
};

__device__ __forceinline__ float row_rs(const GemmParams& p, int row) {
  const float* st = p.row_stats + static_cast<long long>(row) * p.row_stats_n;
  float s = 0.f;
  for (int c0 = 0; c0 < p.row_stats_n; c0 += 8) {
    float t[8];
#pragma unroll
    for (int j = 0; j < 8; ++j) t[j] = (c0 + j < p.row_stats_n) ? __ldg(st + c0 + j) : 0.f;
#pragma unroll
    for (int j = 0; j < 8; ++j)
      if (c0 + j < p.row_stats_n) s += t[j];
  }
  return rsqrtf(fmaf(s, p.inv_norm_dim, p.norm_eps));
}

constexpr int GEMM_BM = 128;
constexpr int GEMM_BK = 64;
constexpr int GEMM_THREADS = 256;
constexpr int kEpiBufBytes = 4096;

template <int BN>
struct GemmCfg {
  static constexpr int kStageBytesA = GEMM_BM * GEMM_BK * 2;
  static constexpr int kStageBytesB = BN * GEMM_BK * 2;
  static constexpr int kStageBytes = kStageBytesA + kStageBytesB;
  static constexpr int kStages = (BN == 256) ? 4 : (BN == 128 ? 6 : 8);
  static constexpr int kTmemCols = 2 * BN;
  static constexpr int kEpiBytes = 4 * 2 * kEpiBufBytes;
  static constexpr int kBarBytes = 256;
  static constexpr int kSmemBytes = kStages * kStageBytes + kEpiBytes + kBarBytes + 1024;
};

__device__ __forceinline__ float gelu_tanh_f(float x) {
  const float x2 = x * x;
  const float inner = fmaf(x2, 0.7978845608028654f * 0.044715f, 0.7978845608028654f);
  const float u = x * inner;
  float t;
  asm("tanh.approx.f32 %0, %1;" : "=f"(t) : "f"(u));
  const float hx = 0.5f * x;
  return fmaf(hx, t, hx);
}

__device__ __forceinline__ uint32_t pack_bf16x2(float lo, float hi) {
  __nv_bfloat162 h = __floats2bfloat162_rn(lo, hi);
  return *reinterpret_cast<uint32_t*>(&h);
}

struct EpiRegs {
  float bias[64];
  float rc[32], rs[32];
  int rope_pos = -1;
  int buf_sel = 0;
};

template <int BN>
__device__ __forceinline__ void epi_load_bias(const GemmParams& p, int n0, float (&b)[64]) {
#pragma unroll
  for (int j = 0; j < 64; j += 4) {
    float4 b4 = make_float4(0.f, 0.f, 0.f, 0.f);
    if (n0 + j < p.N) b4 = __ldg(reinterpret_cast<const float4*>(p.bias + n0 + j));
    b[j] = b4.x; b[j + 1] = b4.y; b[j + 2] = b4.z; b[j + 3] = b4.w;
  }
}

template <int BN, int RPW = 32>
__device__ __forceinline__ void gemm_epilogue_slab(const GemmParams& p, const CUtensorMap* map_out_p, uint32_t tmem_acc,
                                                   int row_base, int n_base, int q, int lane, uint8_t* my_bufs,
                                                   EpiRegs& st, uint64_t* ready_bar, uint32_t ready_parity) {
  const int g = row_base + q * RPW + (lane < RPW ? lane : 0);
  const int grp = g / p.grp_in;
  const int r = g - grp * p.grp_in;
  const bool row_ok = (lane < RPW) && (g < p.M) && (r < p.grp_valid);
  const long long obase = static_cast<long long>(grp) * p.grp_stride + p.grp_off + static_cast<long long>(r) * p.ldo;
  const bool has_bias = p.bias != nullptr;
  if (has_bias) epi_load_bias<BN>(p, n_base, st.bias);
  const float rs = (p.row_stats != nullptr && g < p.M) ? row_rs(p, g) : 1.0f;
  if (p.rope_period > 0) {
    const int pos = p.rope_offset + r % p.rope_period;
    if (pos != st.rope_pos) {
      st.rope_pos = pos;
#pragma unroll
      for (int j = 0; j < 32; ++j) {
        st.rc[j] = __ldg(p.rope_cos + static_cast<long long>(j) * p.rope_ld + pos);
        st.rs[j] = __ldg(p.rope_sin + static_cast<long long>(j) * p.rope_ld + pos);
      }
    }
  }
  mbar_wait(ready_bar, ready_parity);
  tc_fence_after();

#pragma unroll 1
  for (int c = 0; c < BN / 64; ++c) {
    const int n0 = n_base + c * 64;
    if (n0 >= p.N) break;
    uint32_t raw0[32], raw1[32];
    const uint32_t taddr = tmem_acc + (static_cast<uint32_t>(q * 32) << 16) + c * 64;
    tmem_ld_32x32b_x32(taddr, raw0);
    tmem_ld_32x32b_x32(taddr + 32, raw1);
    tmem_ld_wait();
    float v[64];
#pragma unroll
    for (int j = 0; j < 32; ++j) {
      v[j] = __uint_as_float(raw0[j]);
      v[32 + j] = __uint_as_float(raw1[j]);
    }
    if (p.row_stats != nullptr && has_bias) {
#pragma unroll
      for (int j = 0; j < 64; ++j) v[j] = fmaf(v[j], rs, st.bias[j]);
      if (c + 1 < BN / 64 && n0 + 64 < p.N) epi_load_bias<BN>(p, n0 + 64, st.bias);
    } else if (p.row_stats != nullptr) {
#pragma unroll
      for (int j = 0; j < 64; ++j) v[j] = __fmul_rn(v[j], rs);
    } else if (has_bias) {
#pragma unroll
      for (int j = 0; j < 64; ++j) v[j] += st.bias[j];
      if (c + 1 < BN / 64 && n0 + 64 < p.N) epi_load_bias<BN>(p, n0 + 64, st.bias);
    }
    if (p.act == ACT_GELU_TANH) {
#pragma unroll
      for (int j = 0; j < 64; ++j) v[j] = gelu_tanh_f(v[j]);
    }
    if (p.rope_period > 0 && n0 < p.rope_cols) {
#pragma unroll
      for (int j = 0; j < 32; ++j) {
        const float x1 = v[j], x2 = v[32 + j];
        v[j] = x1 * st.rc[j] - x2 * st.rs[j];
        v[32 + j] = x1 * st.rs[j] + x2 * st.rc[j];
      }
    }
    if (p.tma_store) {
      const int row0 = row_base + q * 32;
      const int sw = lane & 7;
      if (p.out_mode == OUT_BF16) {
        uint8_t* buf = my_bufs + st.buf_sel * kEpiBufBytes;
        if (lane == 0) tma_wait_group_read<1>();
        __syncwarp();
#pragma unroll
        for (int j = 0; j < 8; ++j) {
          uint4 w;
          w.x = pack_bf16x2(v[8 * j], v[8 * j + 1]);
          w.y = pack_bf16x2(v[8 * j + 2], v[8 * j + 3]);
          w.z = pack_bf16x2(v[8 * j + 4], v[8 * j + 5]);
          w.w = pack_bf16x2(v[8 * j + 6], v[8 * j + 7]);
          *reinterpret_cast<uint4*>(buf + lane * 128 + ((j ^ sw) << 4)) = w;
        }
        fence_proxy_async_smem();
        __syncwarp();
        if (lane == 0) {
          tma_store_2d(map_out_p, buf, n0, row0);
          tma_commit_group();
        }
        st.buf_sel ^= 1;
      } else {
#pragma unroll
        for (int half = 0; half < 2; ++half) {
          if (n0 + 32 * half < p.N) {
            uint8_t* buf = my_bufs + st.buf_sel * kEpiBufBytes;
            if (lane == 0) tma_wait_group_read<1>();
            __syncwarp();
#pragma unroll
            for (int j = 0; j < 8; ++j) {
              const float* vv = v + 32 * half + 4 * j;
              *reinterpret_cast<float4*>(buf + lane * 128 + ((j ^ sw) << 4)) = make_float4(vv[0], vv[1], vv[2], vv[3]);
            }
            fence_proxy_async_smem();
            __syncwarp();
            if (lane == 0) {
              if (p.out_mode == OUT_F32_RESIDUAL) tma_reduce_add_2d(map_out_p, buf, n0 + 32 * half, row0);
              else tma_store_2d(map_out_p, buf, n0 + 32 * half, row0);
              tma_commit_group();
            }
            st.buf_sel ^= 1;
          }
        }
      }
    } else if (row_ok) {
      if (p.out_mode == OUT_BF16) {
        __nv_bfloat16* o = reinterpret_cast<__nv_bfloat16*>(p.out) + obase + n0;
#pragma unroll
        for (int j = 0; j < 64; j += 8) {
          if (n0 + j < p.N) {
            uint4 w;
            w.x = pack_bf16x2(v[j], v[j + 1]);
            w.y = pack_bf16x2(v[j + 2], v[j + 3]);
            w.z = pack_bf16x2(v[j + 4], v[j + 5]);
            w.w = pack_bf16x2(v[j + 6], v[j + 7]);
            *reinterpret_cast<uint4*>(o + j) = w;
          }
        }
      } else {
        float* o = reinterpret_cast<float*>(p.out) + obase + n0;
        if (p.xb_out != nullptr) {
          const long long orow = (p.grp_in == INT_MAX) ? g : static_cast<long long>(grp) * p.grp_valid + r;
          __nv_bfloat16* xb = p.xb_out + orow * p.N + n0;
          float gam[64];
#pragma unroll
          for (int j = 0; j < 64; j += 4) {
            float4 ga = make_float4(0.f, 0.f, 0.f, 0.f);
            if (n0 + j < p.N) ga = __ldg(reinterpret_cast<const float4*>(p.xb_gamma + n0 + j));
            gam[j] = ga.x; gam[j + 1] = ga.y; gam[j + 2] = ga.z; gam[j + 3] = ga.w;
          }
          if (p.out_mode == OUT_F32_RESIDUAL) {
#pragma unroll
            for (int j = 0; j < 64; j += 4) {
              if (n0 + j < p.N) {
                const float4 a = *reinterpret_cast<const float4*>(o + j);
                v[j] = __fadd_rn(v[j], a.x); v[j + 1] = __fadd_rn(v[j + 1], a.y); v[j + 2] = __fadd_rn(v[j + 2], a.z); v[j + 3] = __fadd_rn(v[j + 3], a.w);
              }
            }
          }
          float ss = 0.f;
#pragma unroll
          for (int j = 0; j < 64; j += 8) {
            if (n0 + j < p.N) {
              *reinterpret_cast<float4*>(o + j) = make_float4(v[j], v[j + 1], v[j + 2], v[j + 3]);
              *reinterpret_cast<float4*>(o + j + 4) = make_float4(v[j + 4], v[j + 5], v[j + 6], v[j + 7]);
#pragma unroll
              for (int e = 0; e < 8; ++e) ss = fmaf(v[j + e], v[j + e], ss);
              uint4 w;
              w.x = pack_bf16x2(__fmul_rn(v[j], gam[j]), __fmul_rn(v[j + 1], gam[j + 1]));
              w.y = pack_bf16x2(__fmul_rn(v[j + 2], gam[j + 2]), __fmul_rn(v[j + 3], gam[j + 3]));
              w.z = pack_bf16x2(__fmul_rn(v[j + 4], gam[j + 4]), __fmul_rn(v[j + 5], gam[j + 5]));
              w.w = pack_bf16x2(__fmul_rn(v[j + 6], gam[j + 6]), __fmul_rn(v[j + 7], gam[j + 7]));
              *reinterpret_cast<uint4*>(xb + j) = w;
            }
          }
          p.stat_out[orow * ((p.N + 63) / 64) + (n0 >> 6)] = ss;
        } else if (p.out_mode == OUT_F32_RESIDUAL) {
#pragma unroll
          for (int j = 0; j < 64; j += 4) {
            if (n0 + j < p.N) {
              float4 x = *reinterpret_cast<const float4*>(o + j);
              x.x += v[j]; x.y += v[j + 1]; x.z += v[j + 2]; x.w += v[j + 3];
              *reinterpret_cast<float4*>(o + j) = x;
            }
          }
        } else {
#pragma unroll
          for (int j = 0; j < 64; j += 4) {
            if (n0 + j < p.N) {
              *reinterpret_cast<float4*>(o + j) = make_float4(v[j], v[j + 1], v[j + 2], v[j + 3]);
            }
          }
        }
      }
    }
  }
}

enum : int { EPI_GENERIC = 0, EPI_ROPE_BF16 = 1, EPI_GELU_BF16 = 2, EPI_RESID_F32 = 3, EPI_RESID_NORM = 4 };

__device__ __forceinline__ void named_bar_sync(int id, int nthreads) {
  asm volatile("bar.sync %0, %1;" ::"r"(id), "r"(nthreads) : "memory");
}
__device__ __forceinline__ void reg_fence32(uint32_t (&v)[32]) {
  asm volatile(""
               : "+r"(v[0]), "+r"(v[1]), "+r"(v[2]), "+r"(v[3]), "+r"(v[4]), "+r"(v[5]), "+r"(v[6]), "+r"(v[7]),
                 "+r"(v[8]), "+r"(v[9]), "+r"(v[10]), "+r"(v[11]), "+r"(v[12]), "+r"(v[13]), "+r"(v[14]), "+r"(v[15]),
                 "+r"(v[16]), "+r"(v[17]), "+r"(v[18]), "+r"(v[19]), "+r"(v[20]), "+r"(v[21]), "+r"(v[22]), "+r"(v[23]),
                 "+r"(v[24]), "+r"(v[25]), "+r"(v[26]), "+r"(v[27]), "+r"(v[28]), "+r"(v[29]), "+r"(v[30]), "+r"(v[31])
               :
               : "memory");
}

struct EpiFastRegs {
  float rc[32], rs[32];
  int rope_pos = -1;
  int buf_sel = 0;
  float row_scale = 1.0f;
  uint32_t xphase = 0;
};

__device__ __forceinline__ float4 lds_f4(const float* smem_ptr) {
  float4 v;
  asm volatile("ld.shared.v4.f32 {%0, %1, %2, %3}, [%4];" : "=f"(v.x), "=f"(v.y), "=f"(v.z), "=f"(v.w) : "r"(smem_u32(smem_ptr)));
  return v;
}
__device__ __forceinline__ void sts_u4(void* smem_ptr, uint4 w) {
  asm volatile("st.shared.v4.b32 [%0], {%1, %2, %3, %4};" ::"r"(smem_u32(smem_ptr)), "r"(w.x), "r"(w.y), "r"(w.z), "r"(w.w) : "memory");
}

template <int EPI>
__device__ __forceinline__ void epi_fast_chunk(const GemmParams& p, const CUtensorMap* map_out_p, uint32_t (&lo)[32],
                                               uint32_t (&hi)[32], const float* sb ,
                                               int n0, int row0, int lane, uint8_t* my_bufs, EpiFastRegs& st) {
  float v[64];
#pragma unroll
  for (int j = 0; j < 32; ++j) {
    v[j] = __uint_as_float(lo[j]);
    v[32 + j] = __uint_as_float(hi[j]);
  }
  if (p.one != 0) {
#pragma unroll
    if (p.row_stats != nullptr) {
      const float rsc = st.row_scale;
#pragma unroll
      for (int j = 0; j < 32; j += 4) {
        const float4 b0 = lds_f4(sb + j);
        const float4 b1 = lds_f4(sb + 32 + j);
        v[j] = fmaf(v[j], rsc, b0.x); v[j + 1] = fmaf(v[j + 1], rsc, b0.y); v[j + 2] = fmaf(v[j + 2], rsc, b0.z); v[j + 3] = fmaf(v[j + 3], rsc, b0.w);
        v[32 + j] = fmaf(v[32 + j], rsc, b1.x); v[32 + j + 1] = fmaf(v[32 + j + 1], rsc, b1.y);
        v[32 + j + 2] = fmaf(v[32 + j + 2], rsc, b1.z); v[32 + j + 3] = fmaf(v[32 + j + 3], rsc, b1.w);
      }
    } else {
#pragma unroll
      for (int j = 0; j < 32; j += 4) {
        const float4 b0 = lds_f4(sb + j);
        const float4 b1 = lds_f4(sb + 32 + j);
        v[j] += b0.x; v[j + 1] += b0.y; v[j + 2] += b0.z; v[j + 3] += b0.w;
        v[32 + j] += b1.x; v[32 + j + 1] += b1.y; v[32 + j + 2] += b1.z; v[32 + j + 3] += b1.w;
      }
    }
    if (EPI == EPI_GELU_BF16) {
#pragma unroll
      for (int j = 0; j < 64; ++j) v[j] = gelu_tanh_f(v[j]);
    }
    if (EPI == EPI_ROPE_BF16) {
      if (n0 < p.rope_cols) {
#pragma unroll
        for (int j = 0; j < 32; ++j) {
          const float x1 = v[j], x2 = v[32 + j];
          v[j] = x1 * st.rc[j] - x2 * st.rs[j];
          v[32 + j] = x1 * st.rs[j] + x2 * st.rc[j];
        }
      }
    }
  }
  const int sw = lane & 7;
  if (EPI == EPI_RESID_F32) {
#pragma unroll
    for (int half = 0; half < 2; ++half) {
      uint8_t* buf = my_bufs + st.buf_sel * kEpiBufBytes;
      if (lane == 0) tma_wait_group_read<1>();
      __syncwarp();
#pragma unroll
      for (int j = 0; j < 8; ++j) {
        const float* vv = v + 32 * half + 4 * j;
        sts_u4(buf + lane * 128 + ((j ^ sw) << 4), make_uint4(__float_as_uint(vv[0]), __float_as_uint(vv[1]), __float_as_uint(vv[2]),
                                                               __float_as_uint(vv[3])));
      }
      fence_proxy_async_smem();
      __syncwarp();
      if (lane == 0) {
        tma_reduce_add_2d(map_out_p, buf, n0 + 32 * half, row0);
        tma_commit_group();
      }
      st.buf_sel ^= 1;
    }
  } else {
    uint8_t* buf = my_bufs + st.buf_sel * kEpiBufBytes;
    if (lane == 0) tma_wait_group_read<1>();
    __syncwarp();
#pragma unroll
    for (int j = 0; j < 8; ++j) {
      uint4 w;
      w.x = pack_bf16x2(v[8 * j], v[8 * j + 1]);
      w.y = pack_bf16x2(v[8 * j + 2], v[8 * j + 3]);
      w.z = pack_bf16x2(v[8 * j + 4], v[8 * j + 5]);
      w.w = pack_bf16x2(v[8 * j + 6], v[8 * j + 7]);
      sts_u4(buf + lane * 128 + ((j ^ sw) << 4), w);
    }
    fence_proxy_async_smem();
    __syncwarp();
    if (lane == 0) {
      tma_store_2d(map_out_p, buf, n0, row0);
      tma_commit_group();
    }
    st.buf_sel ^= 1;
  }
}

template <int BN, int EPI>
__device__ __forceinline__ void gemm_epilogue_slab_fast(const GemmParams& p, const CUtensorMap* map_out_p, uint32_t tmem_acc,
                                                        int row_base, int n_base, int q, int lane, uint8_t* my_bufs,
                                                        float* sbias , EpiFastRegs& st,
                                                        uint64_t* ready_bar, uint32_t ready_parity) {
  static_assert(BN % 128 == 0, "fast epilogue: chunk pairs");
  named_bar_sync(1, 128);
  {
    const int i = q * 32 + lane;
#pragma unroll
    for (int u = 0; u < BN / 128; ++u) {
      const float bv = __ldg(p.bias + n_base + i * (BN / 128) + u);
      asm volatile("st.shared.f32 [%0], %1;" ::"r"(smem_u32(sbias + i * (BN / 128) + u)), "f"(bv) : "memory");
    }
  }
  if (p.row_stats != nullptr) {
    const int g = row_base + q * 32 + lane;
    st.row_scale = g < p.M ? row_rs(p, g) : 1.0f;
  }
  if (EPI == EPI_ROPE_BF16) {
    if (n_base < p.rope_cols) {
      const int g = row_base + q * 32 + lane;
      const int r = g % p.grp_in;
      const int pos = p.rope_offset + r % p.rope_period;
      if (pos != st.rope_pos) {
        st.rope_pos = pos;
#pragma unroll
        for (int j = 0; j < 32; ++j) {
          st.rc[j] = __ldg(p.rope_cos + static_cast<long long>(j) * p.rope_ld + pos);
          st.rs[j] = __ldg(p.rope_sin + static_cast<long long>(j) * p.rope_ld + pos);
        }
      }
    }
  }
  named_bar_sync(1, 128);
  mbar_wait(ready_bar, ready_parity);
  tc_fence_after();

  const int row0 = row_base + q * 32;
  const uint32_t tbase = tmem_acc + (static_cast<uint32_t>(q * 32) << 16);
  uint32_t a_lo[32], a_hi[32], b_lo[32], b_hi[32];
  tmem_ld_32x32b_x32(tbase, a_lo);
  tmem_ld_32x32b_x32(tbase + 32, a_hi);
  tmem_ld_wait();
  reg_fence32(a_lo);
  reg_fence32(a_hi);
#pragma unroll
  for (int c = 0; c < BN / 64; c += 2) {
    tmem_ld_32x32b_x32(tbase + (c + 1) * 64, b_lo);
    tmem_ld_32x32b_x32(tbase + (c + 1) * 64 + 32, b_hi);
    reg_fence32(a_lo);
    reg_fence32(a_hi);
    epi_fast_chunk<EPI>(p, map_out_p, a_lo, a_hi, sbias + c * 64, n_base + c * 64, row0, lane, my_bufs, st);
    tmem_ld_wait();
    reg_fence32(b_lo);
    reg_fence32(b_hi);
    if (c + 2 < BN / 64) {
      tmem_ld_32x32b_x32(tbase + (c + 2) * 64, a_lo);
      tmem_ld_32x32b_x32(tbase + (c + 2) * 64 + 32, a_hi);
    }
    reg_fence32(b_lo);
    reg_fence32(b_hi);
    epi_fast_chunk<EPI>(p, map_out_p, b_lo, b_hi, sbias + (c + 1) * 64, n_base + (c + 1) * 64, row0, lane, my_bufs, st);
    if (c + 2 < BN / 64) {
      tmem_ld_wait();
      reg_fence32(a_lo);
      reg_fence32(a_hi);
    }
  }
}

template <int BN>
__device__ __forceinline__ void gemm_epilogue_slab_resid_norm(const GemmParams& p, const CUtensorMap* map_x, const CUtensorMap* map_xb,
                                                              uint32_t tmem_acc, int row_base, int n_base, int q, int lane,
                                                              uint8_t* wbuf , uint64_t* xbar ,
                                                              float* sbias , EpiFastRegs& st,
                                                              uint64_t* ready_bar, uint32_t ready_parity) {
  static_assert(BN % 128 == 0, "chunk pairs");
  named_bar_sync(1, 128);
  {
    const int i = q * 32 + lane;
#pragma unroll
    for (int u = 0; u < BN / 128; ++u) {
      const int n = i * (BN / 128) + u;
      asm volatile("st.shared.f32 [%0], %1;" ::"r"(smem_u32(sbias + n)), "f"(__ldg(p.bias + n_base + n)) : "memory");
      asm volatile("st.shared.f32 [%0], %1;" ::"r"(smem_u32(sbias + BN + n)), "f"(__ldg(p.xb_gamma + n_base + n)) : "memory");
    }
  }
  const int row0 = row_base + q * 32;
  const int g = row0 + lane;
  uint8_t* xb0 = wbuf;
  uint8_t* bf0 = wbuf + 4 * kEpiBufBytes;
  if (lane == 0) {
    tma_wait_group_read<0>();
#pragma unroll
    for (int set = 0; set < 2; ++set) {
      mbar_arrive_expect_tx(&xbar[set], 2 * kEpiBufBytes);
      tma_load_2d(xb0 + (set * 2) * kEpiBufBytes, map_x, &xbar[set], n_base + set * 64, row0);
      tma_load_2d(xb0 + (set * 2 + 1) * kEpiBufBytes, map_x, &xbar[set], n_base + set * 64 + 32, row0);
    }
  }
  named_bar_sync(1, 128);
  mbar_wait(ready_bar, ready_parity);
  tc_fence_after();
  const uint32_t tbase = tmem_acc + (static_cast<uint32_t>(q * 32) << 16);
  const int sw = lane & 7;
  const int nst = p.N >> 6;
#pragma unroll 1
  for (int c = 0; c < BN / 64; ++c) {
    const int set = c & 1;
    const int n0 = n_base + c * 64;
    uint32_t lo[32], hi[32];
    tmem_ld_32x32b_x32(tbase + c * 64, lo);
    tmem_ld_32x32b_x32(tbase + c * 64 + 32, hi);
    tmem_ld_wait();
    mbar_wait(&xbar[set], (st.xphase >> set) & 1u);
    st.xphase ^= (1u << set);
    float v[64];
    const float* sb = sbias + c * 64;
#pragma unroll
    for (int hf = 0; hf < 2; ++hf) {
      uint8_t* xbox = xb0 + (set * 2 + hf) * kEpiBufBytes + lane * 128;
#pragma unroll
      for (int j = 0; j < 8; ++j) {
        const float4 xo = lds_f4(reinterpret_cast<const float*>(xbox + ((j ^ sw) << 4)));
        const float4 bb = lds_f4(sb + hf * 32 + 4 * j);
        const uint32_t* a = (hf == 0 ? lo : hi) + 4 * j;
        float* vv = v + hf * 32 + 4 * j;
        vv[0] = __fadd_rn(__fadd_rn(__uint_as_float(a[0]), bb.x), xo.x);
        vv[1] = __fadd_rn(__fadd_rn(__uint_as_float(a[1]), bb.y), xo.y);
        vv[2] = __fadd_rn(__fadd_rn(__uint_as_float(a[2]), bb.z), xo.z);
        vv[3] = __fadd_rn(__fadd_rn(__uint_as_float(a[3]), bb.w), xo.w);
      }
    }
    float ss = 0.f;
#pragma unroll
    for (int j = 0; j < 64; ++j) ss = fmaf(v[j], v[j], ss);
    if (g < p.M) p.stat_out[static_cast<long long>(g) * nst + (n0 >> 6)] = ss;
#pragma unroll
    for (int hf = 0; hf < 2; ++hf) {
      uint8_t* xbox = xb0 + (set * 2 + hf) * kEpiBufBytes + lane * 128;
#pragma unroll
      for (int j = 0; j < 8; ++j) {
        const float* vv = v + hf * 32 + 4 * j;
        sts_u4(xbox + ((j ^ sw) << 4), make_uint4(__float_as_uint(vv[0]), __float_as_uint(vv[1]), __float_as_uint(vv[2]), __float_as_uint(vv[3])));
      }
    }
    if (lane == 0) tma_wait_group_read<0>();
    __syncwarp();
    {
      uint8_t* bbox = bf0 + lane * 128;
      const float* sg = sbias + BN + c * 64;
#pragma unroll
      for (int j = 0; j < 8; ++j) {
        const float4 g0 = lds_f4(sg + 8 * j), g1 = lds_f4(sg + 8 * j + 4);
        uint4 w;
        w.x = pack_bf16x2(__fmul_rn(v[8 * j], g0.x), __fmul_rn(v[8 * j + 1], g0.y));
        w.y = pack_bf16x2(__fmul_rn(v[8 * j + 2], g0.z), __fmul_rn(v[8 * j + 3], g0.w));
        w.z = pack_bf16x2(__fmul_rn(v[8 * j + 4], g1.x), __fmul_rn(v[8 * j + 5], g1.y));
        w.w = pack_bf16x2(__fmul_rn(v[8 * j + 6], g1.z), __fmul_rn(v[8 * j + 7], g1.w));
        sts_u4(bbox + ((j ^ sw) << 4), w);
      }
    }
    fence_proxy_async_smem();
    __syncwarp();
    if (lane == 0) {
      tma_store_2d(map_x, xb0 + (set * 2) * kEpiBufBytes, n0, row0);
      tma_store_2d(map_x, xb0 + (set * 2 + 1) * kEpiBufBytes, n0 + 32, row0);
      tma_store_2d(map_xb, bf0, n0, row0);
      tma_commit_group();
      if (c + 2 < BN / 64) {
        tma_wait_group_read<0>();
        mbar_arrive_expect_tx(&xbar[set], 2 * kEpiBufBytes);
        tma_load_2d(xb0 + (set * 2) * kEpiBufBytes, map_x, &xbar[set], n0 + 128, row0);
        tma_load_2d(xb0 + (set * 2 + 1) * kEpiBufBytes, map_x, &xbar[set], n0 + 128 + 32, row0);
      }
    }
    __syncwarp();
  }
}

template <int BN, int BM = GEMM_BM, int KPS = 1>
__global__ void __launch_bounds__(GEMM_THREADS, 1)
gemm_bf16_sm100_kernel(const __grid_constant__ CUtensorMap map_a, const __grid_constant__ CUtensorMap map_b,
                       const __grid_constant__ CUtensorMap map_out, const GemmParams p) {
  using Cfg = GemmCfg<BN>;
  constexpr int kStagesK = Cfg::kStages / KPS;
  constexpr int kStageBytesK = Cfg::kStageBytes * KPS;
  static_assert(Cfg::kStages % KPS == 0 && kStagesK >= 2, "stage grouping");
  extern __shared__ uint8_t smem_raw[];
  uint8_t* smem = reinterpret_cast<uint8_t*>((reinterpret_cast<uintptr_t>(smem_raw) + 1023) & ~uintptr_t(1023));
  uint8_t* epi_base = smem + Cfg::kStages * Cfg::kStageBytes;
  uint8_t* bar_base = epi_base + Cfg::kEpiBytes;
  uint64_t* full_bar = reinterpret_cast<uint64_t*>(bar_base);
  uint64_t* empty_bar = full_bar + Cfg::kStages;
  uint64_t* tmem_full = empty_bar + Cfg::kStages;
  uint64_t* tmem_empty = tmem_full + 2;
  uint32_t* tmem_ptr = reinterpret_cast<uint32_t*>(tmem_empty + 2);

  const int warp = threadIdx.x >> 5;
  const int lane = threadIdx.x & 31;
  const int m_tiles = (p.M + BM - 1) / BM;
  const int n_tiles = (p.N + BN - 1) / BN;
  const int num_tiles = m_tiles * n_tiles;
  const int num_kb = p.K / GEMM_BK;
  constexpr uint32_t kTxBytes = (BM * GEMM_BK * 2 + Cfg::kStageBytesB) * KPS;

  if (warp == 4 && lane == 0) {
    tma_prefetch_desc(&map_a);
    tma_prefetch_desc(&map_b);
    if (p.tma_store) tma_prefetch_desc(&map_out);
  }
  if (warp == 5 && lane == 0) {
    for (int s = 0; s < kStagesK; ++s) {
      mbar_init(&full_bar[s], 1);
      mbar_init(&empty_bar[s], 1);
    }
    for (int s = 0; s < 2; ++s) {
      mbar_init(&tmem_full[s], 1);
      mbar_init(&tmem_empty[s], 4);
    }
    fence_mbar_init();
  }
  if (warp == 6) {
    tmem_alloc(tmem_ptr, Cfg::kTmemCols);
    tmem_relinquish();
  }
  pdl_launch_dependents();
  tc_fence_before();
  __syncthreads();
  tc_fence_after();
  const uint32_t tmem_base = *tmem_ptr;
  pdl_wait();

  if (warp == 4) {
    if (lane == 0) {
      int stage = 0;
      uint32_t phase = 0;
      for (int tile = blockIdx.x; tile < num_tiles; tile += gridDim.x) {
        const int m_blk = tile / n_tiles, n_blk = tile % n_tiles;
        for (int kb = 0; kb < num_kb; kb += KPS) {
          mbar_wait(&empty_bar[stage], phase ^ 1);
          mbar_arrive_expect_tx(&full_bar[stage], kTxBytes);
#pragma unroll
          for (int j = 0; j < KPS; ++j) {
            uint8_t* sa = smem + stage * kStageBytesK + j * Cfg::kStageBytes;
            uint8_t* sb = sa + Cfg::kStageBytesA;
            const int k_elem = (kb + j) * GEMM_BK;
            const int row_off = k_elem / p.a_k_wrap;
            const int a_k = k_elem - row_off * p.a_k_wrap;
            tma_load_2d(sa, &map_a, &full_bar[stage], a_k, m_blk * BM + row_off);
            tma_load_2d(sb, &map_b, &full_bar[stage], k_elem, n_blk * BN);
          }
          if (++stage == kStagesK) { stage = 0; phase ^= 1; }
        }
      }
    }
  } else if (warp == 5) {
    if (lane == 0) {
      constexpr uint32_t idesc = umma_idesc_bf16(BM, BN, 0, 0);
      int stage = 0;
      uint32_t phase = 0;
      int it = 0;
      for (int tile = blockIdx.x; tile < num_tiles; tile += gridDim.x, ++it) {
        const int acc = it & 1;
        const uint32_t acc_phase = (it >> 1) & 1;
        mbar_wait(&tmem_empty[acc], acc_phase ^ 1);
        tc_fence_after();
        const uint32_t d_tmem = tmem_base + acc * BN;
        for (int kb = 0; kb < num_kb; kb += KPS) {
          mbar_wait(&full_bar[stage], phase);
          tc_fence_after();
#pragma unroll
          for (int j = 0; j < KPS; ++j) {
            const uint32_t sa = smem_u32(smem + stage * kStageBytesK + j * Cfg::kStageBytes);
            const uint32_t sb = sa + Cfg::kStageBytesA;
            const uint64_t adesc = umma_smem_desc_sw128(sa, 1024, 16);
            const uint64_t bdesc = umma_smem_desc_sw128(sb, 1024, 16);
#pragma unroll
            for (int k = 0; k < GEMM_BK / 16; ++k) {
              umma_bf16_ss(d_tmem, adesc + 2 * k, bdesc + 2 * k, idesc, (kb | j | k) != 0);
            }
          }
          umma_commit(&empty_bar[stage]);
          if (++stage == kStagesK) { stage = 0; phase ^= 1; }
        }
        umma_commit(&tmem_full[acc]);
      }
    }
  } else if (warp < 4) {
    const int q = warp;
    uint8_t* my_bufs = epi_base + q * 2 * kEpiBufBytes;
    EpiRegs st;
    int it = 0;
    for (int tile = blockIdx.x; tile < num_tiles; tile += gridDim.x, ++it) {
      const int m_blk = tile / n_tiles, n_blk = tile % n_tiles;
      const int acc = it & 1;
      const uint32_t acc_phase = (it >> 1) & 1;
      gemm_epilogue_slab<BN, BM / 4>(p, &map_out, tmem_base + acc * BN, m_blk * BM, n_blk * BN, q, lane, my_bufs, st,
                                     &tmem_full[acc], acc_phase);
      tc_fence_before();
      __syncwarp();
      if (lane == 0) mbar_arrive(&tmem_empty[acc]);
    }
    if (p.tma_store && lane == 0) tma_wait_group_read<0>();
  }

  __syncwarp();
  tc_fence_before();
  __syncthreads();
  if (warp == 6) {
    tc_fence_after();
    tmem_dealloc(tmem_base, Cfg::kTmemCols);
  }
}


template <int BN, int EPI = EPI_GENERIC>
struct Gemm2Cfg {
  static constexpr int kStageBytesA = GEMM_BM * GEMM_BK * 2;
  static constexpr int kStageBytesB = (BN / 2) * GEMM_BK * 2;
  static constexpr int kStageBytes = kStageBytesA + kStageBytesB;
  static constexpr int kEpiBytes = (EPI == EPI_RESID_NORM ? 4 * 5 : 4 * 2) * kEpiBufBytes;
  static constexpr int kStages = (EPI == EPI_RESID_NORM ? 131072 : 196608) / kStageBytes;
  static constexpr int kTmemCols = 2 * BN;
  static constexpr int kBarBytes = 256;
  static constexpr int kBiasBytes = (EPI == EPI_RESID_NORM ? 2 : 1) * BN * 4;
  static constexpr int kSmemBytes = kStages * kStageBytes + kEpiBytes + kBarBytes + kBiasBytes + 1024;
  static_assert(kSmemBytes <= 232448, "CTA-pair GEMM exceeds 227 KB of shared memory");
};

template <int BN, int EPI>
__global__ void __cluster_dims__(2, 1, 1) __launch_bounds__(GEMM_THREADS, 1)
gemm2_bf16_sm100_kernel(const __grid_constant__ CUtensorMap map_a, const __grid_constant__ CUtensorMap map_b,
                        const __grid_constant__ CUtensorMap map_out, const __grid_constant__ CUtensorMap map_out2, const GemmParams p) {
  using Cfg = Gemm2Cfg<BN, EPI>;
  extern __shared__ uint8_t smem_raw[];
  uint8_t* smem = reinterpret_cast<uint8_t*>((reinterpret_cast<uintptr_t>(smem_raw) + 1023) & ~uintptr_t(1023));
  uint8_t* epi_base = smem + Cfg::kStages * Cfg::kStageBytes;
  uint8_t* bar_base = epi_base + Cfg::kEpiBytes;
  uint64_t* full_bar = reinterpret_cast<uint64_t*>(bar_base);
  uint64_t* empty_bar = full_bar + Cfg::kStages;
  uint64_t* tmem_full = empty_bar + Cfg::kStages;
  uint64_t* tmem_empty = tmem_full + 2;
  uint64_t* xbar = tmem_empty + 2;
  uint32_t* tmem_ptr = reinterpret_cast<uint32_t*>(xbar + 8);
  float* sbias = reinterpret_cast<float*>(bar_base + Cfg::kBarBytes);

  const int warp = threadIdx.x >> 5;
  const int lane = threadIdx.x & 31;
  const uint32_t rank = cluster_ctarank();
  const int pair = blockIdx.x >> 1, num_pairs = gridDim.x >> 1;
  const int m_tiles = (p.M + 2 * GEMM_BM - 1) / (2 * GEMM_BM);
  const int n_tiles = (p.N + BN - 1) / BN;
  const int num_tiles = m_tiles * n_tiles;
  const int num_kb = p.K / GEMM_BK;

  if (warp == 4 && lane == 0) {
    tma_prefetch_desc(&map_a);
    tma_prefetch_desc(&map_b);
    if (p.tma_store) tma_prefetch_desc(&map_out);
    if (EPI == EPI_RESID_NORM) tma_prefetch_desc(&map_out2);
  }
  if (warp == 5 && lane == 0) {
    for (int s = 0; s < Cfg::kStages; ++s) {
      mbar_init(&full_bar[s], 2);
      mbar_init(&empty_bar[s], 1);
    }
    for (int s = 0; s < 2; ++s) {
      mbar_init(&tmem_full[s], 1);
      mbar_init(&tmem_empty[s], 8);
    }
    for (int s = 0; s < 8; ++s) mbar_init(&xbar[s], 1);
    fence_mbar_init();
  }
  if (warp == 6) {
    tmem_alloc_pair(tmem_ptr, Cfg::kTmemCols);
    tmem_relinquish_pair();
  }
  pdl_launch_dependents();
  tc_fence_before();
  __syncthreads();
  cluster_sync_all();
  tc_fence_after();
  const uint32_t tmem_base = *tmem_ptr;
  pdl_wait();

  if (warp == 4) {
    if (lane == 0) {
      int stage = 0;
      uint32_t phase = 0;
      for (int tile = pair; tile < num_tiles; tile += num_pairs) {
        const int m_blk = tile / n_tiles, n_blk = tile % n_tiles;
        for (int kb = 0; kb < num_kb; ++kb) {
          mbar_wait(&empty_bar[stage], phase ^ 1);
          uint8_t* sa = smem + stage * Cfg::kStageBytes;
          uint8_t* sb = sa + Cfg::kStageBytesA;
          const uint32_t leader_full = mapa_shared(smem_u32(&full_bar[stage]), 0);
          if (rank == 0) mbar_arrive_expect_tx(&full_bar[stage], 2 * Cfg::kStageBytes);
          else mbar_arrive_cluster(leader_full);
          const int k_elem = kb * GEMM_BK;
          const int row_off = k_elem / p.a_k_wrap;
          const int a_k = k_elem - row_off * p.a_k_wrap;
          tma_load_2d_pair(sa, &map_a, leader_full, a_k, m_blk * 2 * GEMM_BM + rank * GEMM_BM + row_off);
          tma_load_2d_pair(sb, &map_b, leader_full, k_elem, n_blk * BN + rank * (BN / 2));
          if (++stage == Cfg::kStages) { stage = 0; phase ^= 1; }
        }
      }
    }
  } else if (warp == 5) {
    if (lane == 0 && rank == 0) {
      constexpr uint32_t idesc = umma_idesc_bf16(2 * GEMM_BM, BN, 0, 0);
      int stage = 0;
      uint32_t phase = 0;
      int it = 0;
      for (int tile = pair; tile < num_tiles; tile += num_pairs, ++it) {
        const int acc = it & 1;
        const uint32_t acc_phase = (it >> 1) & 1;
        mbar_wait(&tmem_empty[acc], acc_phase ^ 1);
        tc_fence_after();
        const uint32_t d_tmem = tmem_base + acc * BN;
        for (int kb = 0; kb < num_kb; ++kb) {
          mbar_wait(&full_bar[stage], phase);
          tc_fence_after();
          const uint32_t sa = smem_u32(smem + stage * Cfg::kStageBytes);
          const uint32_t sb = sa + Cfg::kStageBytesA;
          const uint64_t adesc = umma_smem_desc_sw128(sa, 1024, 16);
          const uint64_t bdesc = umma_smem_desc_sw128(sb, 1024, 16);
#pragma unroll
          for (int k = 0; k < GEMM_BK / 16; ++k) umma_bf16_ss_pair(d_tmem, adesc + 2 * k, bdesc + 2 * k, idesc, (kb | k) != 0);
          umma_commit_pair(&empty_bar[stage], 3);
          if (++stage == Cfg::kStages) { stage = 0; phase ^= 1; }
        }
        umma_commit_pair(&tmem_full[acc], 3);
      }
    }
  } else if (warp < 4) {
    const int q = warp;
    uint8_t* my_bufs = epi_base + q * (EPI == EPI_RESID_NORM ? 5 : 2) * kEpiBufBytes;
    typename std::conditional<EPI == EPI_GENERIC, EpiRegs, EpiFastRegs>::type st;
    int it = 0;
    for (int tile = pair; tile < num_tiles; tile += num_pairs, ++it) {
      const int m_blk = tile / n_tiles, n_blk = tile % n_tiles;
      const int acc = it & 1;
      const uint32_t acc_phase = (it >> 1) & 1;
      if constexpr (EPI == EPI_GENERIC) {
        gemm_epilogue_slab<BN>(p, &map_out, tmem_base + acc * BN, m_blk * 2 * GEMM_BM + rank * GEMM_BM, n_blk * BN, q, lane,
                               my_bufs, st, &tmem_full[acc], acc_phase);
      } else if constexpr (EPI == EPI_RESID_NORM) {
        gemm_epilogue_slab_resid_norm<BN>(p, &map_out, &map_out2, tmem_base + acc * BN, m_blk * 2 * GEMM_BM + rank * GEMM_BM,
                                          n_blk * BN, q, lane, my_bufs, xbar + 2 * q, sbias, st, &tmem_full[acc], acc_phase);
      } else {
        gemm_epilogue_slab_fast<BN, EPI>(p, &map_out, tmem_base + acc * BN, m_blk * 2 * GEMM_BM + rank * GEMM_BM, n_blk * BN, q,
                                         lane, my_bufs, sbias, st, &tmem_full[acc], acc_phase);
      }
      tc_fence_before();
      __syncwarp();
      if (lane == 0) mbar_arrive_cluster(mapa_shared(smem_u32(&tmem_empty[acc]), 0));
    }
    if (p.tma_store && lane == 0) tma_wait_group_read<0>();
  }

  __syncwarp();
  tc_fence_before();
  __syncthreads();
  cluster_sync_all();
  if (warp == 6) {
    tc_fence_after();
    tmem_dealloc_pair(tmem_base, Cfg::kTmemCols);
  }
}

}
```

### realtime-codec-agent_b200/csrc/ptx_sm100.cuh

```cuda
#pragma once
#include <cuda.h>
#include <cuda_bf16.h>
#include <cuda_runtime.h>
#include <stdint.h>

namespace mc {

__device__ __forceinline__ uint32_t smem_u32(const void* p) {
  return static_cast<uint32_t>(__cvta_generic_to_shared(p));
}

__device__ __forceinline__ float fmax3(float a, float b, float c) {
  float r;
  asm("max.f32 %0, %1, %2, %3;" : "=f"(r) : "f"(a), "f"(b), "f"(c));
  return r;
}

__device__ __forceinline__ uint32_t elect_one() {
  uint32_t pred = 0;
  asm volatile(
      "{\n"
      ".reg .b32 rx;\n"
      ".reg .pred px;\n"
      "elect.sync rx|px, 0xffffffff;\n"
      "selp.u32 %0, 1, 0, px;\n"
      "}\n"
      : "=r"(pred));
  return pred;
}

__device__ __forceinline__ void pdl_launch_dependents() { asm volatile("griddepcontrol.launch_dependents;" ::: "memory"); }
#ifndef MC_TRACE
__device__ __forceinline__ void pdl_wait() { asm volatile("griddepcontrol.wait;" ::: "memory"); }
#define MC_TRACE_DECL
#define MC_TRACE_MARK(ph)
#define MC_TRACE_FLUSH
#else
static __device__ unsigned long long* g_mc_trace = nullptr;
static __device__ unsigned int g_mc_trace_cap = 0;
static __device__ unsigned int g_mc_trace_n = 0;
__device__ __forceinline__ unsigned long long mc_globaltimer() {
  unsigned long long t;
  asm volatile("mov.u64 %0, %%globaltimer;" : "=l"(t));
  return t;
}
__device__ __forceinline__ void pdl_wait() {
  if (threadIdx.x == 0 && g_mc_trace != nullptr) {
    const unsigned long long t0 = mc_globaltimer();
    asm volatile("griddepcontrol.wait;" ::: "memory");
    const unsigned long long t1 = mc_globaltimer();
    const unsigned int slot = atomicAdd(&g_mc_trace_n, 1u);
    if (slot < g_mc_trace_cap) {
      unsigned long long* r = g_mc_trace + 4ull * slot;
      r[0] = (static_cast<unsigned long long>(gridDim.x * gridDim.y) << 32) | (blockIdx.x + blockIdx.y * gridDim.x);
      r[1] = blockDim.x;
      r[2] = t0;
      r[3] = t1;
    }
  } else {
    asm volatile("griddepcontrol.wait;" ::: "memory");
  }
}
struct McTraceMarks {
  unsigned long long t[16];
  unsigned int mask = 0;
};
#define MC_TRACE_DECL McTraceMarks mc_tm_
#define MC_TRACE_MARK(ph) do { if (threadIdx.x == 0 && blockIdx.x == 0) { mc_tm_.t[ph] = mc_globaltimer(); mc_tm_.mask |= 1u << (ph); } } while (0)
#define MC_TRACE_FLUSH mc_trace_flush(mc_tm_)
__device__ __forceinline__ void mc_trace_flush(const McTraceMarks& m) {
  if (threadIdx.x == 0 && blockIdx.x == 0 && g_mc_trace != nullptr) {
#pragma unroll
    for (int ph = 0; ph < 16; ++ph) {
      if (!(m.mask & (1u << ph))) continue;
      const unsigned int slot = atomicAdd(&g_mc_trace_n, 1u);
      if (slot < g_mc_trace_cap) {
        unsigned long long* r = g_mc_trace + 4ull * slot;
        r[0] = static_cast<unsigned long long>(gridDim.x) << 32;
        r[1] = 100000u + ph;
        r[2] = m.t[ph];
        r[3] = m.t[ph];
      }
    }
  }
}
#endif

__device__ __forceinline__ void mbar_init(uint64_t* bar, uint32_t count) {
  asm volatile("mbarrier.init.shared::cta.b64 [%0], %1;" ::"r"(smem_u32(bar)), "r"(count) : "memory");
}
__device__ __forceinline__ void fence_mbar_init() {
  asm volatile("fence.mbarrier_init.release.cluster;" ::: "memory");
}
__device__ __forceinline__ void fence_proxy_async_smem() {
  asm volatile("fence.proxy.async.shared::cta;" ::: "memory");
}
__device__ __forceinline__ void mbar_arrive_expect_tx(uint64_t* bar, uint32_t bytes) {
  asm volatile("mbarrier.arrive.expect_tx.shared::cta.b64 _, [%0], %1;" ::"r"(smem_u32(bar)), "r"(bytes)
               : "memory");
}
__device__ __forceinline__ void mbar_arrive(uint64_t* bar) {
  asm volatile("mbarrier.arrive.shared::cta.b64 _, [%0];" ::"r"(smem_u32(bar)) : "memory");
}
__device__ __forceinline__ uint32_t mbar_try_wait(uint64_t* bar, uint32_t parity) {
  uint32_t ok;
  asm volatile(
      "{\n"
      ".reg .pred p;\n"
      "mbarrier.try_wait.parity.shared::cta.b64 p, [%1], %2;\n"
      "selp.u32 %0, 1, 0, p;\n"
      "}\n"
      : "=r"(ok)
      : "r"(smem_u32(bar)), "r"(parity)
      : "memory");
  return ok;
}
__device__ __forceinline__ void mbar_wait(uint64_t* bar, uint32_t parity) {
  if (mbar_try_wait(bar, parity)) return;
  const long long t0 = clock64();
  while (!mbar_try_wait(bar, parity)) {
    if (clock64() - t0 > 4000000000LL) {
      printf("mbar_wait timeout: block %d thread %d bar %u parity %u\n", blockIdx.x, threadIdx.x,
             smem_u32(bar), parity);
      __trap();
    }
  }
}

__device__ __forceinline__ void tma_prefetch_desc(const CUtensorMap* m) {
  asm volatile("prefetch.tensormap [%0];" ::"l"(reinterpret_cast<uint64_t>(m)) : "memory");
}
__device__ __forceinline__ void tma_load_2d(void* smem_dst, const CUtensorMap* m, uint64_t* bar, int c0, int c1) {
  asm volatile(
      "cp.async.bulk.tensor.2d.shared::cluster.global.mbarrier::complete_tx::bytes [%0], [%1, {%3, %4}], [%2];"
      ::"r"(smem_u32(smem_dst)), "l"(reinterpret_cast<uint64_t>(m)), "r"(smem_u32(bar)), "r"(c0), "r"(c1)
      : "memory");
}
__device__ __forceinline__ void tma_load_2d_hint(void* smem_dst, const CUtensorMap* m, uint64_t* bar, int c0,
                                                 int c1, uint64_t policy) {
  asm volatile(
      "cp.async.bulk.tensor.2d.shared::cluster.global.mbarrier::complete_tx::bytes.L2::cache_hint"
      " [%0], [%1, {%3, %4}], [%2], %5;"
      ::"r"(smem_u32(smem_dst)), "l"(reinterpret_cast<uint64_t>(m)), "r"(smem_u32(bar)), "r"(c0), "r"(c1),
      "l"(policy)
      : "memory");
}
__device__ __forceinline__ void tma_store_2d(const CUtensorMap* m, const void* smem_src, int c0, int c1) {
  asm volatile("cp.async.bulk.tensor.2d.global.shared::cta.bulk_group [%0, {%2, %3}], [%1];" ::"l"(
                   reinterpret_cast<uint64_t>(m)),
               "r"(smem_u32(smem_src)), "r"(c0), "r"(c1)
               : "memory");
}
__device__ __forceinline__ void tma_reduce_add_2d(const CUtensorMap* m, const void* smem_src, int c0, int c1) {
  asm volatile("cp.reduce.async.bulk.tensor.2d.global.shared::cta.add.bulk_group [%0, {%2, %3}], [%1];" ::"l"(
                   reinterpret_cast<uint64_t>(m)),
               "r"(smem_u32(smem_src)), "r"(c0), "r"(c1)
               : "memory");
}
__device__ __forceinline__ void l2_prefetch_bulk(const void* gptr, uint32_t bytes) {
  asm volatile("cp.async.bulk.prefetch.L2.global [%0], %1;" ::"l"(reinterpret_cast<uint64_t>(gptr)), "r"(bytes) : "memory");
}
__device__ __forceinline__ void tma_commit_group() { asm volatile("cp.async.bulk.commit_group;" ::: "memory"); }
template <int N>
__device__ __forceinline__ void tma_wait_group_read() {
  asm volatile("cp.async.bulk.wait_group.read %0;" ::"n"(N) : "memory");
}
template <int N>
__device__ __forceinline__ void tma_wait_group() {
  asm volatile("cp.async.bulk.wait_group %0;" ::"n"(N) : "memory");
}
constexpr uint64_t kEvictNormal = 0x1000000000000000ull;
constexpr uint64_t kEvictFirst = 0x12F0000000000000ull;
constexpr uint64_t kEvictLast = 0x14F0000000000000ull;

__device__ __forceinline__ uint32_t cluster_ctarank() {
  uint32_t r;
  asm volatile("mov.u32 %0, %%cluster_ctarank;" : "=r"(r));
  return r;
}
__device__ __forceinline__ void cluster_sync_all() {
  asm volatile("barrier.cluster.arrive.release.aligned;\n\tbarrier.cluster.wait.acquire.aligned;" ::: "memory");
}
__device__ __forceinline__ uint32_t mapa_shared(uint32_t cta_addr, uint32_t cta_rank) {
  uint32_t r;
  asm volatile("mapa.shared::cluster.u32 %0, %1, %2;" : "=r"(r) : "r"(cta_addr), "r"(cta_rank));
  return r;
}
__device__ __forceinline__ void mbar_arrive_cluster(uint32_t cluster_addr) {
  asm volatile("mbarrier.arrive.shared::cluster.b64 _, [%0];" ::"r"(cluster_addr) : "memory");
}
__device__ __forceinline__ void tma_load_2d_pair(void* smem_dst, const CUtensorMap* m, uint32_t mbar_cluster_addr, int c0,
                                                 int c1) {
  asm volatile(
      "cp.async.bulk.tensor.2d.cta_group::2.shared::cluster.global.mbarrier::complete_tx::bytes [%0], [%1, {%3, %4}], [%2];"
      ::"r"(smem_u32(smem_dst)), "l"(reinterpret_cast<uint64_t>(m)), "r"(mbar_cluster_addr), "r"(c0), "r"(c1)
      : "memory");
}

__device__ __forceinline__ void tmem_alloc(uint32_t* smem_result, uint32_t ncols) {
  asm volatile("tcgen05.alloc.cta_group::1.sync.aligned.shared::cta.b32 [%0], %1;" ::"r"(smem_u32(smem_result)),
               "r"(ncols)
               : "memory");
}
__device__ __forceinline__ void tmem_relinquish() {
  asm volatile("tcgen05.relinquish_alloc_permit.cta_group::1.sync.aligned;" ::: "memory");
}
__device__ __forceinline__ void tmem_dealloc(uint32_t taddr, uint32_t ncols) {
  asm volatile("tcgen05.dealloc.cta_group::1.sync.aligned.b32 %0, %1;" ::"r"(taddr), "r"(ncols) : "memory");
}
__device__ __forceinline__ void tc_fence_before() { asm volatile("tcgen05.fence::before_thread_sync;" ::: "memory"); }
__device__ __forceinline__ void tc_fence_after() { asm volatile("tcgen05.fence::after_thread_sync;" ::: "memory"); }

__device__ __forceinline__ void umma_bf16_ss(uint32_t tmem_d, uint64_t adesc, uint64_t bdesc, uint32_t idesc,
                                             uint32_t accumulate) {
  asm volatile(
      "{\n"
      ".reg .pred p;\n"
      "setp.ne.b32 p, %4, 0;\n"
      "tcgen05.mma.cta_group::1.kind::f16 [%0], %1, %2, %3, p;\n"
      "}\n" ::"r"(tmem_d),
      "l"(adesc), "l"(bdesc), "r"(idesc), "r"(accumulate)
      : "memory");
}
__device__ __forceinline__ void umma_commit(uint64_t* bar) {
  asm volatile("tcgen05.commit.cta_group::1.mbarrier::arrive::one.shared::cluster.b64 [%0];" ::"r"(smem_u32(bar))
               : "memory");
}

__device__ __forceinline__ void tmem_alloc_pair(uint32_t* smem_result, uint32_t ncols) {
  asm volatile("tcgen05.alloc.cta_group::2.sync.aligned.shared::cta.b32 [%0], %1;" ::"r"(smem_u32(smem_result)),
               "r"(ncols)
               : "memory");
}
__device__ __forceinline__ void tmem_relinquish_pair() {
  asm volatile("tcgen05.relinquish_alloc_permit.cta_group::2.sync.aligned;" ::: "memory");
}
__device__ __forceinline__ void tmem_dealloc_pair(uint32_t taddr, uint32_t ncols) {
  asm volatile("tcgen05.dealloc.cta_group::2.sync.aligned.b32 %0, %1;" ::"r"(taddr), "r"(ncols) : "memory");
}
__device__ __forceinline__ void umma_bf16_ss_pair(uint32_t tmem_d, uint64_t adesc, uint64_t bdesc, uint32_t idesc,
                                                  uint32_t accumulate) {
  const uint32_t z = 0;
  asm volatile(
      "{\n"
      ".reg .pred p;\n"
      "setp.ne.b32 p, %4, 0;\n"
      "tcgen05.mma.cta_group::2.kind::f16 [%0], %1, %2, %3, {%5, %5, %5, %5, %5, %5, %5, %5}, p;\n"
      "}\n" ::"r"(tmem_d),
      "l"(adesc), "l"(bdesc), "r"(idesc), "r"(accumulate), "r"(z)
      : "memory");
}
__device__ __forceinline__ void umma_commit_pair(uint64_t* bar, uint16_t cta_mask) {
  asm volatile(
      "tcgen05.commit.cta_group::2.mbarrier::arrive::one.shared::cluster.multicast::cluster.b64 [%0], %1;" ::"r"(
          smem_u32(bar)),
      "h"(cta_mask)
      : "memory");
}

__device__ __forceinline__ void tmem_ld_32x32b_x32(uint32_t taddr, uint32_t (&v)[32]) {
  asm volatile(
      "tcgen05.ld.sync.aligned.32x32b.x32.b32 "
      "{%0, %1, %2, %3, %4, %5, %6, %7, %8, %9, %10, %11, %12, %13, %14, %15, "
      "%16, %17, %18, %19, %20, %21, %22, %23, %24, %25, %26, %27, %28, %29, %30, %31}, [%32];"
      : "=r"(v[0]), "=r"(v[1]), "=r"(v[2]), "=r"(v[3]), "=r"(v[4]), "=r"(v[5]), "=r"(v[6]), "=r"(v[7]),
        "=r"(v[8]), "=r"(v[9]), "=r"(v[10]), "=r"(v[11]), "=r"(v[12]), "=r"(v[13]), "=r"(v[14]), "=r"(v[15]),
        "=r"(v[16]), "=r"(v[17]), "=r"(v[18]), "=r"(v[19]), "=r"(v[20]), "=r"(v[21]), "=r"(v[22]), "=r"(v[23]),
        "=r"(v[24]), "=r"(v[25]), "=r"(v[26]), "=r"(v[27]), "=r"(v[28]), "=r"(v[29]), "=r"(v[30]), "=r"(v[31])
      : "r"(taddr)
      : "memory");
}
__device__ __forceinline__ void tmem_ld_32x32b_x16(uint32_t taddr, uint32_t (&v)[16]) {
  asm volatile(
      "tcgen05.ld.sync.aligned.32x32b.x16.b32 "
      "{%0, %1, %2, %3, %4, %5, %6, %7, %8, %9, %10, %11, %12, %13, %14, %15}, [%16];"
      : "=r"(v[0]), "=r"(v[1]), "=r"(v[2]), "=r"(v[3]), "=r"(v[4]), "=r"(v[5]), "=r"(v[6]), "=r"(v[7]),
        "=r"(v[8]), "=r"(v[9]), "=r"(v[10]), "=r"(v[11]), "=r"(v[12]), "=r"(v[13]), "=r"(v[14]), "=r"(v[15])
      : "r"(taddr)
      : "memory");
}
__device__ __forceinline__ void tmem_ld_wait() { asm volatile("tcgen05.wait::ld.sync.aligned;" ::: "memory"); }
__device__ __forceinline__ void tmem_st_32x32b_x16(uint32_t taddr, const uint32_t (&v)[16]) {
  asm volatile(
      "tcgen05.st.sync.aligned.32x32b.x16.b32 [%0], "
      "{%1, %2, %3, %4, %5, %6, %7, %8, %9, %10, %11, %12, %13, %14, %15, %16};"
      ::"r"(taddr), "r"(v[0]), "r"(v[1]), "r"(v[2]), "r"(v[3]), "r"(v[4]), "r"(v[5]), "r"(v[6]), "r"(v[7]), "r"(v[8]),
      "r"(v[9]), "r"(v[10]), "r"(v[11]), "r"(v[12]), "r"(v[13]), "r"(v[14]), "r"(v[15])
      : "memory");
}
__device__ __forceinline__ void tmem_st_wait() { asm volatile("tcgen05.wait::st.sync.aligned;" ::: "memory"); }
__device__ __forceinline__ void umma_bf16_ts(uint32_t tmem_d, uint32_t tmem_a, uint64_t bdesc, uint32_t idesc,
                                             uint32_t accumulate) {
  asm volatile(
      "{\n"
      ".reg .pred p;\n"
      "setp.ne.b32 p, %4, 0;\n"
      "tcgen05.mma.cta_group::1.kind::f16 [%0], [%1], %2, %3, p;\n"
      "}\n" ::"r"(tmem_d),
      "r"(tmem_a), "l"(bdesc), "r"(idesc), "r"(accumulate)
      : "memory");
}

__device__ __forceinline__ uint64_t umma_smem_desc_sw128(uint32_t smem_addr, uint32_t sbo_bytes,
                                                         uint32_t lbo_bytes) {
  uint64_t d = 0;
  d |= static_cast<uint64_t>((smem_addr & 0x3FFFF) >> 4);
  d |= static_cast<uint64_t>((lbo_bytes >> 4) & 0x3FFF) << 16;
  d |= static_cast<uint64_t>((sbo_bytes >> 4) & 0x3FFF) << 32;
  d |= static_cast<uint64_t>(1) << 46;
  d |= static_cast<uint64_t>(2) << 61;
  return d;
}

__host__ __device__ constexpr uint32_t umma_idesc_bf16(uint32_t M, uint32_t N, uint32_t a_mn_major,
                                                       uint32_t b_mn_major) {
  return (1u << 4) | (1u << 7) | (1u << 10) | (a_mn_major << 15) | (b_mn_major << 16) | ((N >> 3) << 17) |
         ((M >> 4) << 24);
}

}
```

Measured before the change: 5635.

## Use eight epilogue warps with register rebalancing in fast-path pair GEMM

Adds a template parameter that doubles the epilogue warps from four to eight in the CTA-pair GEMM for the fast epilogue modes (RoPE, GELU, residual F32). Each warp handles half the accumulator columns, and setmaxnreg moves registers from the producer and MMA warps to the epilogue warps. The aim is to drain TMEM and write output faster so the MMA warp waits less for a free accumulator. In exchange, the extra epilogue buffers take shared memory away from pipeline stages, and the change adds opt-in cycle-counter instrumentation and an occupancy debug query.

```diff
diff --git a/include/magicodec_b200.h b/include/magicodec_b200.h
--- a/include/magicodec_b200.h
+++ b/include/magicodec_b200.h
@@ -64,6 +64,8 @@
                    mc_stream_t stream);
 
 int64_t mc_debug_trace(mc_handle* h, void* dev_buf, int64_t capacity_records);
+int mc_debug_cycles(mc_handle* h, int64_t* out, int32_t n);
+int mc_debug_max_active_clusters(mc_handle* h, int32_t cluster_size, int32_t* out);
 
 enum { MC_PCM_U8 = 0, MC_PCM_S16 = 1, MC_PCM_S24 = 2, MC_PCM_S32 = 3, MC_PCM_F32 = 4, MC_PCM_F64 = 5, MC_PCM_ULAW = 6, MC_PCM_ALAW = 7 };
 int mc_op_pcm_to_f32(mc_handle* h, const void* pcm, int32_t format, int32_t big_endian, int32_t channels, int64_t frames,
diff --git a/realtime-codec-agent_b200/_native.py b/realtime-codec-agent_b200/_native.py
--- a/realtime-codec-agent_b200/_native.py
+++ b/realtime-codec-agent_b200/_native.py
@@ -41,6 +41,8 @@
     "mc_codebook": (C.c_int, [_P, _P, _P]),
     "mc_launch_count": (_I64, [_P]),
     "mc_debug_trace": (_I64, [_P, _P, _I64]),
+    "mc_debug_cycles": (C.c_int, [_P, _P, _I32]),
+    "mc_debug_max_active_clusters": (C.c_int, [_P, _I32, C.POINTER(_I32)]),
     "mc_set_debug_impl": (C.c_int, [_P, _I32, _I32]),
     "mc_set_option": (C.c_int, [_P, C.c_char_p, _I32]),
     "mc_profile_begin": (C.c_int, [_P]),
diff --git a/realtime-codec-agent_b200/build.py b/realtime-codec-agent_b200/build.py
--- a/realtime-codec-agent_b200/build.py
+++ b/realtime-codec-agent_b200/build.py
@@ -32,10 +32,13 @@
     raise RuntimeError("nvcc not found; the B200 engine cannot be built")
 
 
-def build(force: bool = False, verbose: bool = False, trace: bool = False) -> str:
-    digest = _sources_digest() + ("+trace" if trace else "")
-    lib_path = LIB_PATH.replace(".so", "_trace.so") if trace else LIB_PATH
-    stamp = _STAMP + ("_trace" if trace else "")
+def build(force: bool = False, verbose: bool = False, trace: bool = False, cycles: bool = False) -> str:
+    if trace and cycles:
+        raise ValueError("build: trace and cycles are separate diagnostic builds")
+    variant = "_trace" if trace else ("_cycles" if cycles else "")
+    digest = _sources_digest() + ("+" + variant[1:] if variant else "")
+    lib_path = LIB_PATH.replace(".so", variant + ".so")
+    stamp = _STAMP + variant
     if not force and os.path.isfile(lib_path) and os.path.isfile(stamp):
         with open(stamp) as f:
             if f.read().strip() == digest:
@@ -43,7 +46,7 @@
     cmd = [
         nvcc_path(), "-std=c++17", "-O3", "-lineinfo",
         "-gencode", "arch=compute_100a,code=sm_100a",
-        "-Xcompiler", "-fPIC,-O2,-Wall", "-shared", *(["-DMC_TRACE"] if trace else []),
+        "-Xcompiler", "-fPIC,-O2,-Wall", "-shared", *(["-DMC_TRACE"] if trace else []), *(["-DMC_CYCLES"] if cycles else []),
         "-Xptxas", "-v" if verbose else "-O3",
         "-o", lib_path, os.path.join(CSRC, "engine.cu"), os.path.join(CSRC, "audio_decode.cpp"),
         "-lcudart",
@@ -60,7 +63,7 @@
 
 def main(argv=None) -> None:
     argv = sys.argv[1:] if argv is None else argv
-    print(build(force="--force" in argv, verbose="-v" in argv, trace="--trace" in argv))
+    print(build(force="--force" in argv, verbose="-v" in argv, trace="--trace" in argv, cycles="--cycles" in argv))
 
 
 if __name__ == "__main__":
diff --git a/realtime-codec-agent_b200/csrc/engine.cu b/realtime-codec-agent_b200/csrc/engine.cu
--- a/realtime-codec-agent_b200/csrc/engine.cu
+++ b/realtime-codec-agent_b200/csrc/engine.cu
@@ -66,15 +66,23 @@
   return MC_OK;
 }
 
-template <int EPI>
+template <int EPI, int NEPI = 4>
 int launch_gemm_pair_epi(mc_handle* h, const GemmParams& p, const CUtensorMap* ma, const CUtensorMap* mb,
                          const CUtensorMap* mo, const CUtensorMap* mo2, int pairs, cudaStream_t stream) {
   constexpr int BN = 256;
-  MC_TRY(mc_allow_smem(h, gemm2_bf16_sm100_kernel<BN, EPI>, Gemm2Cfg<BN, EPI>::kSmemBytes));
-  mc_launch(h, gemm2_bf16_sm100_kernel<BN, EPI>, dim3(2 * pairs), dim3(GEMM_THREADS), Gemm2Cfg<BN, EPI>::kSmemBytes, stream, *ma, *mb,
+  using Cfg = Gemm2Cfg<BN, EPI, NEPI>;
+  MC_TRY(mc_allow_smem(h, gemm2_bf16_sm100_kernel<BN, EPI, NEPI>, Cfg::kSmemBytes));
+  mc_launch(h, gemm2_bf16_sm100_kernel<BN, EPI, NEPI>, dim3(2 * pairs), dim3(Cfg::kThreads), Cfg::kSmemBytes, stream, *ma, *mb,
             *mo, *mo2, p);
   MC_LAUNCH_CHECK(h, "gemm2_bf16_sm100_kernel");
   return MC_OK;
+}
+
+template <int EPI>
+int launch_gemm_pair_fast(mc_handle* h, const GemmParams& p, const CUtensorMap* ma, const CUtensorMap* mb,
+                          const CUtensorMap* mo, int pairs, cudaStream_t stream) {
+  if (h->gemm_epi8) return launch_gemm_pair_epi<EPI, 8>(h, p, ma, mb, mo, mo, pairs, stream);
+  return launch_gemm_pair_epi<EPI, 4>(h, p, ma, mb, mo, mo, pairs, stream);
 }
 
 int launch_gemm_pair(mc_handle* h, const GemmCall& c, cudaStream_t stream) {
@@ -110,11 +118,11 @@
   const bool fast_ok = h->fast_epilogue && tma_out && c.bias != nullptr && c.N % BN == 0;
   if (norm_fast) return launch_gemm_pair_epi<EPI_RESID_NORM>(h, p, ma, mb, mo, mo2, pairs, stream);
   if (fast_ok && c.out_mode == OUT_BF16 && c.act == ACT_NONE && c.rope_period > 0 && c.rope_cols % 64 == 0)
-    return launch_gemm_pair_epi<EPI_ROPE_BF16>(h, p, ma, mb, mo, mo2, pairs, stream);
+    return launch_gemm_pair_fast<EPI_ROPE_BF16>(h, p, ma, mb, mo, pairs, stream);
   if (fast_ok && c.out_mode == OUT_BF16 && c.act == ACT_GELU_TANH && c.rope_period == 0)
-    return launch_gemm_pair_epi<EPI_GELU_BF16>(h, p, ma, mb, mo, mo2, pairs, stream);
+    return launch_gemm_pair_fast<EPI_GELU_BF16>(h, p, ma, mb, mo, pairs, stream);
   if (fast_ok && c.out_mode == OUT_F32_RESIDUAL && c.act == ACT_NONE && c.rope_period == 0 && c.xb_out == nullptr)
-    return launch_gemm_pair_epi<EPI_RESID_F32>(h, p, ma, mb, mo, mo2, pairs, stream);
+    return launch_gemm_pair_fast<EPI_RESID_F32>(h, p, ma, mb, mo, pairs, stream);
   return launch_gemm_pair_epi<EPI_GENERIC>(h, p, ma, mb, mo, mo2, pairs, stream);
 }
 
@@ -952,6 +960,40 @@
 #endif
 }
 
+int mc_debug_cycles(mc_handle* h, int64_t* out, int32_t n) {
+  if (!h || !out) return MC_ERR_ARG;
+#ifdef MC_CYCLES
+  unsigned long long v[MC_CYC_COUNT] = {};
+  MC_CUDA(h, cudaDeviceSynchronize());
+  MC_CUDA(h, cudaMemcpyFromSymbol(v, g_mc_cyc, sizeof(v)));
+  const unsigned long long zero[MC_CYC_COUNT] = {};
+  MC_CUDA(h, cudaMemcpyToSymbol(g_mc_cyc, zero, sizeof(zero)));
+  for (int i = 0; i < n; ++i) out[i] = i < MC_CYC_COUNT ? (int64_t)v[i] : 0;
+  return MC_OK;
+#else
+  (void)n;
+  return h->fail(MC_ERR_STATE, "mc_debug_cycles: the library was built without -DMC_CYCLES");
+#endif
+}
+
+int mc_debug_max_active_clusters(mc_handle* h, int32_t cluster_size, int32_t* out) {
+  if (!h || !out || cluster_size < 1) return MC_ERR_ARG;
+  auto kernel = gemm_bf16_sm100_kernel<256>;
+  const int smem = Gemm2Cfg<256, EPI_GELU_BF16>::kSmemBytes;
+  MC_TRY(mc_allow_smem(h, kernel, smem));
+  cudaLaunchConfig_t cfg = {};
+  cfg.gridDim = dim3(cluster_size * h->num_sms); cfg.blockDim = dim3(GEMM_THREADS); cfg.dynamicSmemBytes = smem;
+  cudaLaunchAttribute at[1];
+  at[0].id = cudaLaunchAttributeClusterDimension;
+  at[0].val.clusterDim.x = cluster_size; at[0].val.clusterDim.y = 1; at[0].val.clusterDim.z = 1;
+  cfg.attrs = at;
+  cfg.numAttrs = 1;
+  int n = 0;
+  MC_CUDA(h, cudaOccupancyMaxActiveClusters(&n, kernel, &cfg));
+  *out = n;
+  return MC_OK;
+}
+
 int64_t mc_launch_count(const mc_handle* h) { return h ? h->launches : 0; }
 
 int mc_profile_begin(mc_handle* h) {
@@ -985,6 +1027,7 @@
   else if (k == "exact_cut") { h->exact_cut = value != 0; h->tensor_gen++; }
   else if (k == "gemm_pair") h->gemm_pair = value != 0;
   else if (k == "fast_epilogue") h->fast_epilogue = value != 0;
+  else if (k == "gemm_epi8") h->gemm_epi8 = value != 0;
   else if (k == "pdl") h->pdl = value != 0;
   else if (k == "attn_p_tmem") h->attn_p_tmem = value != 0;
   else if (k == "debug_repeat") h->debug_repeat = value;
diff --git a/realtime-codec-agent_b200/csrc/engine_common.cuh b/realtime-codec-agent_b200/csrc/engine_common.cuh
--- a/realtime-codec-agent_b200/csrc/engine_common.cuh
+++ b/realtime-codec-agent_b200/csrc/engine_common.cuh
@@ -61,6 +61,7 @@
   int attn_impl = 0, vq_impl = 0;
   int gemm_pair = 1;
   bool fast_epilogue = true;
+  bool gemm_epi8 = true;
   bool attn_p_tmem = true;
   int split_k = 1;
   bool in_session = false;
diff --git a/realtime-codec-agent_b200/csrc/gemm_sm100.cuh b/realtime-codec-agent_b200/csrc/gemm_sm100.cuh
--- a/realtime-codec-agent_b200/csrc/gemm_sm100.cuh
+++ b/realtime-codec-agent_b200/csrc/gemm_sm100.cuh
@@ -87,6 +87,7 @@
   float rc[32], rs[32];
   int rope_pos = -1;
   int buf_sel = 0;
+  MC_CYC(long long cyc_wait = 0;)
 };
 
 template <int BN>
@@ -122,7 +123,9 @@
       }
     }
   }
+  MC_CYC(const long long cyc_t0 = clock64();)
   mbar_wait(ready_bar, ready_parity);
+  MC_CYC(st.cyc_wait += clock64() - cyc_t0;)
   tc_fence_after();
 
 #pragma unroll 1
@@ -305,6 +308,7 @@
   int buf_sel = 0;
   float row_scale = 1.0f;
   uint32_t xphase = 0;
+  MC_CYC(long long cyc_wait = 0;)
 };
 
 __device__ __forceinline__ float4 lds_f4(const float* smem_ptr) {
@@ -316,7 +320,7 @@
   asm volatile("st.shared.v4.b32 [%0], {%1, %2, %3, %4};" ::"r"(smem_u32(smem_ptr)), "r"(w.x), "r"(w.y), "r"(w.z), "r"(w.w) : "memory");
 }
 
-template <int EPI>
+template <int EPI, int NBUF>
 __device__ __forceinline__ void epi_fast_chunk(const GemmParams& p, const CUtensorMap* map_out_p, uint32_t (&lo)[32],
                                                uint32_t (&hi)[32], const float* sb ,
                                                int n0, int row0, int lane, uint8_t* my_bufs, EpiFastRegs& st) {
@@ -367,7 +371,7 @@
 #pragma unroll
     for (int half = 0; half < 2; ++half) {
       uint8_t* buf = my_bufs + st.buf_sel * kEpiBufBytes;
-      if (lane == 0) tma_wait_group_read<1>();
+      if (lane == 0) tma_wait_group_read<NBUF - 1>();
       __syncwarp();
 #pragma unroll
       for (int j = 0; j < 8; ++j) {
@@ -381,11 +385,11 @@
         tma_reduce_add_2d(map_out_p, buf, n0 + 32 * half, row0);
         tma_commit_group();
       }
-      st.buf_sel ^= 1;
+      if (NBUF > 1) st.buf_sel ^= 1;
     }
   } else {
     uint8_t* buf = my_bufs + st.buf_sel * kEpiBufBytes;
-    if (lane == 0) tma_wait_group_read<1>();
+    if (lane == 0) tma_wait_group_read<NBUF - 1>();
     __syncwarp();
 #pragma unroll
     for (int j = 0; j < 8; ++j) {
@@ -402,23 +406,25 @@
       tma_store_2d(map_out_p, buf, n0, row0);
       tma_commit_group();
     }
-    st.buf_sel ^= 1;
-  }
-}
-
-template <int BN, int EPI>
+    if (NBUF > 1) st.buf_sel ^= 1;
+  }
+}
+
+template <int BN, int EPI, int NEPI, int NBUF>
 __device__ __forceinline__ void gemm_epilogue_slab_fast(const GemmParams& p, const CUtensorMap* map_out_p, uint32_t tmem_acc,
-                                                        int row_base, int n_base, int q, int lane, uint8_t* my_bufs,
+                                                        int row_base, int n_base, int q, int c_first, int lane, uint8_t* my_bufs,
                                                         float* sbias , EpiFastRegs& st,
                                                         uint64_t* ready_bar, uint32_t ready_parity) {
-  static_assert(BN % 128 == 0, "fast epilogue: chunk pairs");
-  named_bar_sync(1, 128);
+  constexpr int NCH = BN / 16 / NEPI;
+  constexpr int kBiasPerThread = BN / (32 * NEPI);
+  static_assert(NCH % 2 == 0 && kBiasPerThread >= 1, "fast epilogue: chunk pairs");
+  named_bar_sync(1, 32 * NEPI);
   {
-    const int i = q * 32 + lane;
-#pragma unroll
-    for (int u = 0; u < BN / 128; ++u) {
-      const float bv = __ldg(p.bias + n_base + i * (BN / 128) + u);
-      asm volatile("st.shared.f32 [%0], %1;" ::"r"(smem_u32(sbias + i * (BN / 128) + u)), "f"(bv) : "memory");
+    const int i = (threadIdx.x >> 5) * 32 + lane;
+#pragma unroll
+    for (int u = 0; u < kBiasPerThread; ++u) {
+      const float bv = __ldg(p.bias + n_base + i * kBiasPerThread + u);
+      asm volatile("st.shared.f32 [%0], %1;" ::"r"(smem_u32(sbias + i * kBiasPerThread + u)), "f"(bv) : "memory");
     }
   }
   if (p.row_stats != nullptr) {
@@ -426,7 +432,7 @@
     st.row_scale = g < p.M ? row_rs(p, g) : 1.0f;
   }
   if (EPI == EPI_ROPE_BF16) {
-    if (n_base < p.rope_cols) {
+    if (n_base + c_first * 64 < p.rope_cols) {
       const int g = row_base + q * 32 + lane;
       const int r = g % p.grp_in;
       const int pos = p.rope_offset + r % p.rope_period;
@@ -440,12 +446,16 @@
       }
     }
   }
-  named_bar_sync(1, 128);
+  named_bar_sync(1, 32 * NEPI);
+  MC_CYC(const long long cyc_t0 = clock64();)
   mbar_wait(ready_bar, ready_parity);
+  MC_CYC(st.cyc_wait += clock64() - cyc_t0;)
   tc_fence_after();
 
   const int row0 = row_base + q * 32;
-  const uint32_t tbase = tmem_acc + (static_cast<uint32_t>(q * 32) << 16);
+  const uint32_t tbase = tmem_acc + (static_cast<uint32_t>(q * 32) << 16) + c_first * 64;
+  const int nb = n_base + c_first * 64;
+  const float* sb = sbias + c_first * 64;
   uint32_t a_lo[32], a_hi[32], b_lo[32], b_hi[32];
   tmem_ld_32x32b_x32(tbase, a_lo);
   tmem_ld_32x32b_x32(tbase + 32, a_hi);
@@ -453,23 +463,23 @@
   reg_fence32(a_lo);
   reg_fence32(a_hi);
 #pragma unroll
-  for (int c = 0; c < BN / 64; c += 2) {
+  for (int c = 0; c < NCH; c += 2) {
     tmem_ld_32x32b_x32(tbase + (c + 1) * 64, b_lo);
     tmem_ld_32x32b_x32(tbase + (c + 1) * 64 + 32, b_hi);
     reg_fence32(a_lo);
     reg_fence32(a_hi);
-    epi_fast_chunk<EPI>(p, map_out_p, a_lo, a_hi, sbias + c * 64, n_base + c * 64, row0, lane, my_bufs, st);
+    epi_fast_chunk<EPI, NBUF>(p, map_out_p, a_lo, a_hi, sb + c * 64, nb + c * 64, row0, lane, my_bufs, st);
     tmem_ld_wait();
     reg_fence32(b_lo);
     reg_fence32(b_hi);
-    if (c + 2 < BN / 64) {
+    if (c + 2 < NCH) {
       tmem_ld_32x32b_x32(tbase + (c + 2) * 64, a_lo);
       tmem_ld_32x32b_x32(tbase + (c + 2) * 64 + 32, a_hi);
     }
     reg_fence32(b_lo);
     reg_fence32(b_hi);
-    epi_fast_chunk<EPI>(p, map_out_p, b_lo, b_hi, sbias + (c + 1) * 64, n_base + (c + 1) * 64, row0, lane, my_bufs, st);
-    if (c + 2 < BN / 64) {
+    epi_fast_chunk<EPI, NBUF>(p, map_out_p, b_lo, b_hi, sb + (c + 1) * 64, nb + (c + 1) * 64, row0, lane, my_bufs, st);
+    if (c + 2 < NCH) {
       tmem_ld_wait();
       reg_fence32(a_lo);
       reg_fence32(a_hi);
@@ -508,7 +518,9 @@
     }
   }
   named_bar_sync(1, 128);
+  MC_CYC(const long long cyc_t0 = clock64();)
   mbar_wait(ready_bar, ready_parity);
+  MC_CYC(st.cyc_wait += clock64() - cyc_t0;)
   tc_fence_after();
   const uint32_t tbase = tmem_acc + (static_cast<uint32_t>(q * 32) << 16);
   const int sw = lane & 7;
@@ -723,13 +735,16 @@
 }
 
 
-template <int BN, int EPI = EPI_GENERIC>
+template <int BN, int EPI = EPI_GENERIC, int NEPI = 4>
 struct Gemm2Cfg {
+  static_assert(NEPI == 4 || (NEPI == 8 && EPI != EPI_GENERIC && EPI != EPI_RESID_NORM), "8 epilogue warps: fast modes only");
+  static constexpr int kThreads = 32 * (NEPI + 4);
   static constexpr int kStageBytesA = GEMM_BM * GEMM_BK * 2;
   static constexpr int kStageBytesB = (BN / 2) * GEMM_BK * 2;
   static constexpr int kStageBytes = kStageBytesA + kStageBytesB;
-  static constexpr int kEpiBytes = (EPI == EPI_RESID_NORM ? 4 * 5 : 4 * 2) * kEpiBufBytes;
-  static constexpr int kStages = (EPI == EPI_RESID_NORM ? 131072 : 196608) / kStageBytes;
+  static constexpr int kEpiBufs = 2;
+  static constexpr int kEpiBytes = (EPI == EPI_RESID_NORM ? 4 * 5 : NEPI * kEpiBufs) * kEpiBufBytes;
+  static constexpr int kStages = (EPI == EPI_RESID_NORM ? 131072 : 196608 + 8 * kEpiBufBytes - kEpiBytes) / kStageBytes;
   static constexpr int kTmemCols = 2 * BN;
   static constexpr int kBarBytes = 256;
   static constexpr int kBiasBytes = (EPI == EPI_RESID_NORM ? 2 : 1) * BN * 4;
@@ -737,11 +752,26 @@
   static_assert(kSmemBytes <= 232448, "CTA-pair GEMM exceeds 227 KB of shared memory");
 };
 
-template <int BN, int EPI>
-__global__ void __cluster_dims__(2, 1, 1) __launch_bounds__(GEMM_THREADS, 1)
+template <uint32_t N> __device__ __forceinline__ void setmaxnreg_inc() { asm volatile("setmaxnreg.inc.sync.aligned.u32 %0;" ::"n"(N)); }
+template <uint32_t N> __device__ __forceinline__ void setmaxnreg_dec() { asm volatile("setmaxnreg.dec.sync.aligned.u32 %0;" ::"n"(N)); }
+
+struct Gemm2Walk {
+  uint32_t rank;
+  int pair, num_pairs, n_tiles, num_tiles, num_kb;
+};
+template <int BN>
+__device__ __forceinline__ Gemm2Walk gemm2_walk(const GemmParams& p) {
+  const int n_tiles = (p.N + BN - 1) / BN;
+  return {cluster_ctarank(), static_cast<int>(blockIdx.x >> 1), static_cast<int>(gridDim.x >> 1), n_tiles,
+          ((p.M + 2 * GEMM_BM - 1) / (2 * GEMM_BM)) * n_tiles, p.K / GEMM_BK};
+}
+
+template <int BN, int EPI, int NEPI>
+__global__ void __cluster_dims__(2, 1, 1) __launch_bounds__(Gemm2Cfg<BN, EPI, NEPI>::kThreads, 1)
 gemm2_bf16_sm100_kernel(const __grid_constant__ CUtensorMap map_a, const __grid_constant__ CUtensorMap map_b,
                         const __grid_constant__ CUtensorMap map_out, const __grid_constant__ CUtensorMap map_out2, const GemmParams p) {
-  using Cfg = Gemm2Cfg<BN, EPI>;
+  using Cfg = Gemm2Cfg<BN, EPI, NEPI>;
+  constexpr int kProducerWarp = NEPI, kMmaWarp = NEPI + 1, kAllocWarp = NEPI + 2;
   extern __shared__ uint8_t smem_raw[];
   uint8_t* smem = reinterpret_cast<uint8_t*>((reinterpret_cast<uintptr_t>(smem_raw) + 1023) & ~uintptr_t(1023));
   uint8_t* epi_base = smem + Cfg::kStages * Cfg::kStageBytes;
@@ -755,33 +785,25 @@
   float* sbias = reinterpret_cast<float*>(bar_base + Cfg::kBarBytes);
 
   const int warp = threadIdx.x >> 5;
-  const int lane = threadIdx.x & 31;
-  const uint32_t rank = cluster_ctarank();
-  const int pair = blockIdx.x >> 1, num_pairs = gridDim.x >> 1;
-  const int m_tiles = (p.M + 2 * GEMM_BM - 1) / (2 * GEMM_BM);
-  const int n_tiles = (p.N + BN - 1) / BN;
-  const int num_tiles = m_tiles * n_tiles;
-  const int num_kb = p.K / GEMM_BK;
-
-  if (warp == 4 && lane == 0) {
+  if (warp == kProducerWarp && threadIdx.x % 32 == 0) {
     tma_prefetch_desc(&map_a);
     tma_prefetch_desc(&map_b);
     if (p.tma_store) tma_prefetch_desc(&map_out);
     if (EPI == EPI_RESID_NORM) tma_prefetch_desc(&map_out2);
   }
-  if (warp == 5 && lane == 0) {
+  if (warp == kMmaWarp && threadIdx.x % 32 == 0) {
     for (int s = 0; s < Cfg::kStages; ++s) {
       mbar_init(&full_bar[s], 2);
       mbar_init(&empty_bar[s], 1);
     }
     for (int s = 0; s < 2; ++s) {
       mbar_init(&tmem_full[s], 1);
-      mbar_init(&tmem_empty[s], 8);
+      mbar_init(&tmem_empty[s], 2 * NEPI);
     }
     for (int s = 0; s < 8; ++s) mbar_init(&xbar[s], 1);
     fence_mbar_init();
   }
-  if (warp == 6) {
+  if (warp == kAllocWarp) {
     tmem_alloc_pair(tmem_ptr, Cfg::kTmemCols);
     tmem_relinquish_pair();
   }
@@ -790,17 +812,23 @@
   __syncthreads();
   cluster_sync_all();
   tc_fence_after();
-  const uint32_t tmem_base = *tmem_ptr;
   pdl_wait();
-
-  if (warp == 4) {
+  constexpr bool kRebalance = NEPI == 8;
+
+  if (warp == kProducerWarp) {
+    if constexpr (kRebalance) setmaxnreg_dec<56>();
+    const auto [rank, pair, num_pairs, n_tiles, num_tiles, num_kb] = gemm2_walk<BN>(p);
+    const int lane = threadIdx.x & 31;
     if (lane == 0) {
+      MC_CYC(long long cyc_empty = 0;)
       int stage = 0;
       uint32_t phase = 0;
       for (int tile = pair; tile < num_tiles; tile += num_pairs) {
         const int m_blk = tile / n_tiles, n_blk = tile % n_tiles;
         for (int kb = 0; kb < num_kb; ++kb) {
+          MC_CYC(const long long t0 = clock64();)
           mbar_wait(&empty_bar[stage], phase ^ 1);
+          MC_CYC(cyc_empty += clock64() - t0;)
           uint8_t* sa = smem + stage * Cfg::kStageBytes;
           uint8_t* sb = sa + Cfg::kStageBytesA;
           const uint32_t leader_full = mapa_shared(smem_u32(&full_bar[stage]), 0);
@@ -814,9 +842,15 @@
           if (++stage == Cfg::kStages) { stage = 0; phase ^= 1; }
         }
       }
-    }
-  } else if (warp == 5) {
+      MC_CYC(atomicAdd(&g_mc_cyc[MC_CYC_PRODUCER_EMPTY], (unsigned long long)cyc_empty);)
+    }
+  } else if (warp == kMmaWarp) {
+    if constexpr (kRebalance) setmaxnreg_dec<56>();
+    const auto [rank, pair, num_pairs, n_tiles, num_tiles, num_kb] = gemm2_walk<BN>(p);
+    const int lane = threadIdx.x & 31;
+    const uint32_t tmem_base = *tmem_ptr;
     if (lane == 0 && rank == 0) {
+      MC_CYC(long long cyc_full = 0, cyc_tmem = 0; const long long cyc_start = clock64(); int cyc_tiles = 0;)
       constexpr uint32_t idesc = umma_idesc_bf16(2 * GEMM_BM, BN, 0, 0);
       int stage = 0;
       uint32_t phase = 0;
@@ -824,11 +858,15 @@
       for (int tile = pair; tile < num_tiles; tile += num_pairs, ++it) {
         const int acc = it & 1;
         const uint32_t acc_phase = (it >> 1) & 1;
+        MC_CYC(long long t0 = clock64();)
         mbar_wait(&tmem_empty[acc], acc_phase ^ 1);
+        MC_CYC(cyc_tmem += clock64() - t0; ++cyc_tiles;)
         tc_fence_after();
         const uint32_t d_tmem = tmem_base + acc * BN;
         for (int kb = 0; kb < num_kb; ++kb) {
+          MC_CYC(t0 = clock64();)
           mbar_wait(&full_bar[stage], phase);
+          MC_CYC(cyc_full += clock64() - t0;)
           tc_fence_after();
           const uint32_t sa = smem_u32(smem + stage * Cfg::kStageBytes);
           const uint32_t sb = sa + Cfg::kStageBytesA;
@@ -841,13 +879,23 @@
         }
         umma_commit_pair(&tmem_full[acc], 3);
       }
-    }
-  } else if (warp < 4) {
-    const int q = warp;
-    uint8_t* my_bufs = epi_base + q * (EPI == EPI_RESID_NORM ? 5 : 2) * kEpiBufBytes;
+      MC_CYC(atomicAdd(&g_mc_cyc[MC_CYC_TILES], (unsigned long long)cyc_tiles);
+             atomicAdd(&g_mc_cyc[MC_CYC_MMA_FULL], (unsigned long long)cyc_full);
+             atomicAdd(&g_mc_cyc[MC_CYC_MMA_TMEM_EMPTY], (unsigned long long)cyc_tmem);
+             atomicAdd(&g_mc_cyc[MC_CYC_MMA_TOTAL], (unsigned long long)(clock64() - cyc_start));)
+    }
+  } else if (warp < NEPI) {
+    if constexpr (kRebalance) setmaxnreg_inc<224>();
+    const auto [rank, pair, num_pairs, n_tiles, num_tiles, num_kb] = gemm2_walk<BN>(p);
+    const int lane = threadIdx.x & 31;
+    const uint32_t tmem_base = *tmem_ptr;
+    const int q = warp & 3;
+    uint8_t* my_bufs = epi_base + warp * (EPI == EPI_RESID_NORM ? 5 : Cfg::kEpiBufs) * kEpiBufBytes;
     typename std::conditional<EPI == EPI_GENERIC, EpiRegs, EpiFastRegs>::type st;
+    MC_CYC(long long cyc_epi = 0; int cyc_tiles = 0;)
     int it = 0;
     for (int tile = pair; tile < num_tiles; tile += num_pairs, ++it) {
+      MC_CYC(const long long t0 = clock64();)
       const int m_blk = tile / n_tiles, n_blk = tile % n_tiles;
       const int acc = it & 1;
       const uint32_t acc_phase = (it >> 1) & 1;
@@ -858,24 +906,33 @@
         gemm_epilogue_slab_resid_norm<BN>(p, &map_out, &map_out2, tmem_base + acc * BN, m_blk * 2 * GEMM_BM + rank * GEMM_BM,
                                           n_blk * BN, q, lane, my_bufs, xbar + 2 * q, sbias, st, &tmem_full[acc], acc_phase);
       } else {
-        gemm_epilogue_slab_fast<BN, EPI>(p, &map_out, tmem_base + acc * BN, m_blk * 2 * GEMM_BM + rank * GEMM_BM, n_blk * BN, q,
-                                         lane, my_bufs, sbias, st, &tmem_full[acc], acc_phase);
+        gemm_epilogue_slab_fast<BN, EPI, NEPI, Cfg::kEpiBufs>(p, &map_out, tmem_base + acc * BN, m_blk * 2 * GEMM_BM + rank * GEMM_BM,
+                                                              n_blk * BN, q, (warp >> 2) * (BN / 16 / NEPI), lane, my_bufs, sbias, st,
+                                                              &tmem_full[acc], acc_phase);
       }
       tc_fence_before();
       __syncwarp();
       if (lane == 0) mbar_arrive_cluster(mapa_shared(smem_u32(&tmem_empty[acc]), 0));
+      MC_CYC(cyc_epi += clock64() - t0; ++cyc_tiles;)
     }
     if (p.tma_store && lane == 0) tma_wait_group_read<0>();
+    MC_CYC(if (lane == 0) {
+      atomicAdd(&g_mc_cyc[MC_CYC_EPI_WAIT], (unsigned long long)st.cyc_wait);
+      atomicAdd(&g_mc_cyc[MC_CYC_EPI_TOTAL], (unsigned long long)cyc_epi);
+      atomicAdd(&g_mc_cyc[MC_CYC_EPI_WARP_TILES], (unsigned long long)cyc_tiles);
+    })
+  } else {
+    if constexpr (kRebalance) setmaxnreg_dec<56>();
   }
 
   __syncwarp();
   tc_fence_before();
   __syncthreads();
   cluster_sync_all();
-  if (warp == 6) {
+  if (warp == kAllocWarp) {
     tc_fence_after();
-    tmem_dealloc_pair(tmem_base, Cfg::kTmemCols);
-  }
-}
-
-}
+    tmem_dealloc_pair(*tmem_ptr, Cfg::kTmemCols);
+  }
+}
+
+}
diff --git a/realtime-codec-agent_b200/csrc/ptx_sm100.cuh b/realtime-codec-agent_b200/csrc/ptx_sm100.cuh
--- a/realtime-codec-agent_b200/csrc/ptx_sm100.cuh
+++ b/realtime-codec-agent_b200/csrc/ptx_sm100.cuh
@@ -86,6 +86,15 @@
 }
 #endif
 
+#ifdef MC_CYCLES
+enum : int { MC_CYC_TILES = 0, MC_CYC_MMA_FULL, MC_CYC_MMA_TMEM_EMPTY, MC_CYC_MMA_TOTAL, MC_CYC_EPI_WAIT, MC_CYC_EPI_TOTAL,
+             MC_CYC_EPI_WARP_TILES, MC_CYC_PRODUCER_EMPTY, MC_CYC_COUNT };
+static __device__ unsigned long long g_mc_cyc[MC_CYC_COUNT];
+#define MC_CYC(...) __VA_ARGS__
+#else
+#define MC_CYC(...)
+#endif
+
 __device__ __forceinline__ void mbar_init(uint64_t* bar, uint32_t count) {
   asm volatile("mbarrier.init.shared::cta.b64 [%0], %1;" ::"r"(smem_u32(bar)), "r"(count) : "memory");
 }
```

Measured after the change: 5563 (median of 6 runs). 0.987x the previous value.
